# SZU-AdvTech-2024/140-ExtDM-Distribution-Extrapolation-Diffusion-Model-for-Video-Prediction

Hardware: AMD Instinct MI355X
Metric: predicted frames/sec/node (DDPM 1000-step) BAIR 64×64 2→28; FVD parity (higher is better)
Workload: dtype fp32 (f16x3 split-MFMA convs + attention, fp32 accumulate); 1 GPU; BAIR 64x64 ch3 2->28 (tp=14 x 2 rounds), DDPM 1000 steps, Unet3D (multi_w_ref wrapper), LFAE encoder + flow-warp decoder, occlusion map off (eval default); bench_config=bair, global_batch=128, batch_per_gpu=128, sampling_steps=1000, rounds=2, parallelism=clip-shard x1 (+gather to rank 0)

## Files before the change

140-extdm-distribution-extrapolation-diffusion-model-for-video-prediction_amd/csrc/conv_x3.hip:

```cpp
#include <algorithm>
#include <cstdlib>

#include "host_util.h"
#include "kernels.h"

#ifndef EXTDM_X3_LIN
#define EXTDM_X3_LIN 2
#endif
#ifndef EXTDM_X3_BUFX
#define EXTDM_X3_BUFX 1
#endif
#ifndef EXTDM_X3_EXP
#define EXTDM_X3_EXP 0
#endif

namespace extdm {

__device__ int g_x3_range;

namespace {

typedef float f32x16 __attribute__((ext_vector_type(16)));
typedef _Float16 h8 __attribute__((ext_vector_type(8)));
typedef __attribute__((address_space(3))) void* lds_ptr_t;

struct X3Args {
  const float* in0; const float* in1;
  long i0b, i0c, i0t, i1b, i1c, i1t;
  int C0, Cin, H, W, T, P;
  const _Float16* w; const float* wscale; int ncgb;
  float* out; long ob, oc, ot; int Cout;
  int TH, NP, nrow_tiles, RS, XPOS;
  int out_bytes, res_bytes;
  int stats_split;
  const _Float16* xop; long xop_cg, xop_hl;
  float* part; int nsplit;
  float* edge;
  int mfast;
  int mtc;
  int in0_bytes, in1_bytes;
  ConvEpi e;
};

__device__ __forceinline__ float act_apply(float v, int act) {
  switch (act) {
    case ACT_RELU: return v > 0.f ? v : 0.f;
    case ACT_GELU: return 0.5f * v * (1.f + erff(v * 0.70710678118654752f));
    case ACT_SILU: return v / (1.f + expf(-v));
    case ACT_SIGMOID: return 1.f / (1.f + expf(-v));
    default: return v;
  }
}

__device__ __forceinline__ void glds16_asm(const void* gsrc, _Float16* lds) {
  const unsigned dst =
      __builtin_amdgcn_readfirstlane((unsigned)(uintptr_t)(__attribute__((address_space(3))) void*)lds);
  unsigned keep;
  asm volatile("s_mov_b32 %0, m0\n\ts_mov_b32 m0, %2\n\ts_nop 0\n\tglobal_load_lds_dwordx4 %1, off\n\ts_mov_b32 m0, %0"
               : "=&s"(keep)
               : "v"(gsrc), "s"(dst)
               : "memory");
}

__device__ __forceinline__ void bld4_asm(__amdgpu_buffer_rsrc_t rs, int voff, float* lds) {
  const unsigned dst =
      __builtin_amdgcn_readfirstlane((unsigned)(uintptr_t)(__attribute__((address_space(3))) void*)lds);
  unsigned keep;
  asm volatile("s_mov_b32 %0, m0\n\ts_mov_b32 m0, %3\n\ts_nop 0\n\tbuffer_load_dword %1, %2, 0 offen lds\n\ts_mov_b32 m0, %0"
               : "=&s"(keep)
               : "v"(voff), "s"(rs), "s"(dst)
               : "memory");
}

template <int KS, int BN> struct XMaxX3;
template <> struct XMaxX3<7, 256> { static constexpr int v = 560; };
template <> struct XMaxX3<3, 256> { static constexpr int v = 576; };
template <> struct XMaxX3<3, 128> { static constexpr int v = 288; };
template <> struct XMaxX3<1, 128> { static constexpr int v = 128; };
template <> struct XMaxX3<1, 256> { static constexpr int v = 256; };
template <> struct XMaxX3<7, 512> { static constexpr int v = 836; };
template <> struct XMaxX3<3, 512> { static constexpr int v = 800; };
template <> struct XMaxX3<5, 512> { static constexpr int v = 800; };
template <> struct XMaxX3<5, 256> { static constexpr int v = 400; };

template <int KS, int KY, int BM, int BN, int NG, int WN, int NW, int XBUF, bool SPAN, int NS, bool XOP = false,
          bool RGN = false, int SPL = 0, bool PH = false, bool WS = false, bool BX = false, int TT = 0>
__global__ __launch_bounds__(NW * 64) __attribute__((amdgpu_waves_per_eu(NW == 4 && KS == 5 ? 2 : 1))) void conv_x3_kernel(X3Args a) {
  constexpr int NT = NW * 64;
  constexpr int PAD = KS / 2;
  constexpr int CIB = 16 * NG;
  constexpr int MT32 = BM / 32;
  constexpr int KT = TT ? 2 : KS;
  constexpr int STEPS = NG * KT;
  constexpr int AH = STEPS * MT32 * 2 * 512;
  constexpr int AHS = KY * AH;
  constexpr int STG = KT / KY;
  static_assert(KT % KY == 0, "KY must divide the taps");
  static_assert(!TT || (KS == 3 && NG == 1 && BX && SPAN && !XOP && !WS && !PH && SPL == 0), "TT: staged 3x3 geometry");
  constexpr int NSLOT = NS;
  constexpr int WM = NW / WN;
  constexpr int TM = BM / (32 * WM);
  constexpr int TN = BN / (32 * WN);
  static_assert(TM >= 1 && TN >= 1 && WM * WN == NW, "bad tile");
  static_assert(!XOP || (NG == 1 && XBUF == 2 && SPAN), "operand input: one group, two X buffers");

  extern __shared__ __attribute__((aligned(16))) _Float16 smx[];
  static_assert(!WS || (NG == 1 && SPAN && SPL != 2 && NW % 2 == 0), "WS: one group, spanning barriers");
  constexpr bool WSR = WS && !XOP;
  constexpr bool LIN = WSR || ((EXTDM_X3_LIN == 1 || (EXTDM_X3_LIN == 2 && KS >= 5)) && NG == 1 && !XOP);
  const int XPL = ((a.XPOS + (LIN ? 1 : 0) + 63) & ~63) * 8;
  const int XLO = (XOP || LIN) ? 2 * XPL : NG * a.XPOS * 16;
  const int XH = 2 * XLO;
  constexpr int XB = WSR ? 1 : XBUF;
  const int RP = (a.XPOS + 63) & ~63;
  _Float16* As0 = smx;
  _Float16* As1 = smx + AHS;
  _Float16* Xs0 = smx + 2 * AHS;
  _Float16* Xs1 = XB == 2 ? Xs0 + XH : Xs0;
  float* const Xr = reinterpret_cast<float*>(Xs0 + XB * XH);

  const int tid = threadIdx.x, lane = tid & 63, wave = tid >> 6;
  const int wm = wave / WN, wn = wave % WN;
  const int h = lane >> 5, lc = lane & 31;
  int tile, mtile;
  if ((KS == 1 || TT == 1) && a.mfast) {
    const int lin = (int)(blockIdx.x + gridDim.x * blockIdx.y), MT = (int)gridDim.y;
    const int k = lin >> 3;
    mtile = k % MT;
    tile = (lin & 7) + 8 * (k / MT);
  } else {
    tile = (KS == 1 || (gridDim.x & 7)) ? (int)blockIdx.x
                                        : (int)((blockIdx.x & 7) * (gridDim.x >> 3) + (blockIdx.x >> 3));
    mtile = blockIdx.y;
  }
  const int plane0 = (tile / a.nrow_tiles) * a.NP;
  const int row0 = (tile % a.nrow_tiles) * a.TH;

  const int THK = a.TH + KS - 1;
  const int tb = (plane0 * (a.H + KS - 1) + row0) * a.RS;
  const int c0 = SPL == 1 ? (int)blockIdx.z * a.ncgb / a.nsplit : 0;
  const int c1 = SPL == 1 ? ((int)blockIdx.z + 1) * a.ncgb / a.nsplit : a.ncgb;
  const int NIT = c1 * STG;
  const _Float16* wt = a.w + (long)mtile * a.ncgb * KT * AH;
  const int tph = TT == 1 ? mtile / a.mtc : 0;
  const int mbase = (TT == 1 ? mtile - tph * a.mtc : mtile) * BM;
  auto in_phase = [&](int cgb) __attribute__((always_inline)) {
    const int ncb = a.ncgb >> 2;
    return (cgb >= ncb) + (cgb >= 2 * ncb) + (cgb >= 3 * ncb);
  };

  int sg[NSLOT], spos[NSLOT], soff0[NSLOT], soff1[NSLOT];
#pragma unroll
  for (int j = 0; j < NSLOT; ++j) {
    const int sl = tid + NT * j;
    sg[j] = -1; spos[j] = 0; soff0[j] = -1; soff1[j] = -1;
    if (sl < a.XPOS * NG) {
      const int g = sl / a.XPOS, pos = sl - g * a.XPOS;
      const int p = pos / (THK * a.RS);
      const int r2 = pos - p * THK * a.RS;
      const int rr = r2 / a.RS, cc = r2 - rr * a.RS;
      const int q = plane0 + p;
      const int iy = row0 + rr - PAD, ix = cc - PAD;
      sg[j] = g; spos[j] = pos;
      if (q < a.P && iy >= 0 && iy < a.H && ix >= 0 && ix < a.W) {
        const int b = q / a.T, t = q - b * a.T;
        const int ip = TT == 2 ? 4 * iy * a.W + 2 * ix : iy * a.W + ix;
        soff0[j] = (int)((long)b * a.i0b + (long)t * a.i0t) + ip;
        soff1[j] = (int)((long)b * a.i1b + (long)t * a.i1t) + ip;
      }
    }
  }
  float xr[NSLOT][16];
  int range_bad = 0;

  const float* const gin0 = a.in0;
  const float* const gin1 = a.in1;
  const long gi0c = a.i0c, gi1c = a.i1c;
  const int gC0 = a.C0, gCin = a.Cin;
  const bool whole = gC0 % 16 == 0 && gCin % CIB == 0;
  const bool bufx = BX || (EXTDM_X3_BUFX && whole && a.in0_bytes > 0);
  const auto rsx0 = __builtin_amdgcn_make_buffer_rsrc(const_cast<float*>(a.in0), 0, a.in0_bytes, 0x00020000);
  const auto rsx1 = __builtin_amdgcn_make_buffer_rsrc(const_cast<float*>(a.in1), 0, a.in1_bytes, 0x00020000);
  auto load_x_exact = [&](int cgb) __attribute__((always_inline)) {
#if EXTDM_X3_EXP & 2
#pragma unroll
    for (int j = 0; j < NSLOT; ++j)
#pragma unroll
      for (int c = 0; c < 16; ++c) xr[j][c] = 0.f;
    return;
#endif
    if (bufx) {
      const int qin = TT == 2 ? in_phase(cgb) : 0;
      const int cbk = TT == 2 ? cgb - qin * (a.ncgb >> 2) : cgb;
      const int poff = TT == 2 ? ((qin >> 1) * 2 * a.W + (qin & 1)) * 4 : 0;
#pragma unroll
      for (int j = 0; j < NSLOT; ++j) {
        const int ci0 = __builtin_amdgcn_readfirstlane(cbk * CIB + (sg[j] < 0 ? 0 : sg[j]) * 16);
        const bool s1 = ci0 >= gC0;
        const int vo = soff0[j] >= 0 ? (s1 ? soff1[j] : soff0[j]) * 4 : 0x40000000;
        const int cb = s1 ? ci0 - gC0 : ci0;
        const int cs4 = (int)(s1 ? gi1c : gi0c) * 4;
#pragma unroll
        for (int c = 0; c < 16; ++c)
          xr[j][c] = __uint_as_float(__builtin_amdgcn_raw_buffer_load_b32(s1 ? rsx1 : rsx0, vo, (cb + c) * cs4 + poff, 0));
      }
      return;
    }
#pragma unroll
    for (int j = 0; j < NSLOT; ++j) {
      const bool pos_ok = soff0[j] >= 0;
      const int o0 = pos_ok ? soff0[j] : 0, o1 = pos_ok ? soff1[j] : 0;
      const int ci0 = cgb * CIB + (sg[j] < 0 ? 0 : sg[j]) * 16;
      if (whole) {
        const bool s1 = ci0 >= gC0;
        const float* bp = s1 ? gin1 + (long)(ci0 - gC0) * gi1c + o1 : gin0 + (long)ci0 * gi0c + o0;
        const long cs = s1 ? gi1c : gi0c;
#pragma unroll
        for (int c = 0; c < 16; ++c) xr[j][c] = bp[c * cs];
        continue;
      }
#pragma unroll
      for (int c = 0; c < 16; ++c) {
        const int ci = ci0 + c;
        const bool s1 = ci >= gC0;
        int cc = s1 ? ci - gC0 : ci;
        const int cmax = s1 ? gCin - gC0 - 1 : gC0 - 1;
        cc = cc > cmax ? cmax : cc;
        const long off = s1 ? (long)cc * gi1c + o1 : (long)cc * gi0c + o0;
        xr[j][c] = (s1 ? gin1 : gin0)[off];
      }
    }
  };
  auto xmask = [&](int j, int cgb, int c) __attribute__((always_inline)) {
    const int ci = cgb * CIB + (sg[j] < 0 ? 0 : sg[j]) * 16 + c;
    return (soff0[j] >= 0 && ci < gCin) ? 1.f : 0.f;
  };
  auto load_x = [&](int cgb) __attribute__((always_inline)) {
    if (SPAN) {
      load_x_exact(cgb);
      return;
    }
#pragma unroll
    for (int j = 0; j < NSLOT; ++j) {
      const int ci0 = cgb * CIB + sg[j] * 16;
      const bool src1 = ci0 >= a.C0;
      const float* base = src1 ? a.in1 + (long)(ci0 - a.C0) * a.i1c : a.in0 + (long)ci0 * a.i0c;
      const int cs = src1 ? (int)a.i1c : (int)a.i0c;
      const int off = src1 ? soff1[j] : soff0[j];
      const int cend = src1 ? a.Cin : a.C0;
      if (off >= 0 && ci0 + 16 <= cend) {
#pragma unroll
        for (int c = 0; c < 16; ++c) xr[j][c] = base[off + c * cs];
      } else {
#pragma unroll
        for (int c = 0; c < 16; ++c) {
          const int ci = ci0 + c;
          float v = 0.f;
          if (soff0[j] >= 0 && ci < a.Cin)
            v = ci < a.C0 ? a.in0[(long)ci * a.i0c + soff0[j]] : a.in1[(long)(ci - a.C0) * a.i1c + soff1[j]];
          xr[j][c] = v;
        }
      }
    }
  };
  _Float16* const xdummy = Xs0 + XB * XH + (WSR ? 2 * 16 * RP : 0);
  auto store_x = [&](_Float16* Xs, int cgb) __attribute__((always_inline)) {
#pragma unroll
    for (int j = 0; j < NSLOT; ++j) {
      if (!SPAN && sg[j] < 0) continue;
      float v[16];
#pragma unroll
      for (int c = 0; c < 16; ++c) {
        float r = xr[j][c];
        if (SPAN) {
          asm volatile("" : "+v"(r));
          if (!bufx) r *= xmask(j, cgb, c);
        }
        v[c] = r;
      }
      unsigned hw[8], lw[8];
      float am = 0.f;
#pragma unroll
      for (int c = 0; c < 8; ++c) {
        split2s(v[2 * c], v[2 * c + 1], hw[c], lw[c]);
        amax2(am, v[2 * c], v[2 * c + 1]);
      }
      range_bad |= am >= 65504.f;
      const h8 hi0 = __builtin_bit_cast(h8, u32x4{hw[0], hw[1], hw[2], hw[3]});
      const h8 hi1 = __builtin_bit_cast(h8, u32x4{hw[4], hw[5], hw[6], hw[7]});
      const h8 lo0 = __builtin_bit_cast(h8, u32x4{lw[0], lw[1], lw[2], lw[3]});
      const h8 lo1 = __builtin_bit_cast(h8, u32x4{lw[4], lw[5], lw[6], lw[7]});
      const bool used = sg[j] >= 0;
      if (LIN) {
        _Float16* d = Xs + (used ? spos[j] : XPL / 8 - 1) * 8;
        *reinterpret_cast<h8*>(d) = hi0;
        *reinterpret_cast<h8*>(d + XPL) = hi1;
        *reinterpret_cast<h8*>(d + 2 * XPL) = lo0;
        *reinterpret_cast<h8*>(d + 3 * XPL) = lo1;
        continue;
      }
      const int sw = (spos[j] >> 3) & 1;
      _Float16* dh = used ? Xs + ((long)sg[j] * a.XPOS + spos[j]) * 16 : xdummy;
      _Float16* dl = used ? dh + XLO : xdummy + 16;
      *reinterpret_cast<h8*>(dh + 8 * sw) = hi0;
      *reinterpret_cast<h8*>(dh + 8 * (sw ^ 1)) = hi1;
      *reinterpret_cast<h8*>(dl + 8 * sw) = lo0;
      *reinterpret_cast<h8*>(dl + 8 * (sw ^ 1)) = lo1;
    }
  };
  constexpr int NPIECE = AHS / 512;
  const int wave_u = __builtin_amdgcn_readfirstlane(wave);
  auto load_a = [&](int it, _Float16* As) {
#if EXTDM_X3_EXP & 8
    return;
#endif
    const _Float16* src = wt + (long)it * AHS;
    if (WS && wave_u >= NW / 2) return;
    for (int pc = wave_u; pc < NPIECE; pc += (WS ? NW / 2 : NW)) {
      if (SPAN) glds16_asm(src + pc * 512 + lane * 8, As + pc * 512);
      else
        __builtin_amdgcn_global_load_lds((const void*)(src + pc * 512 + lane * 8), (lds_ptr_t)(As + pc * 512), 16, 0,
                                         0);
    }
  };

  auto dma_x = [&](int cgb, _Float16* Xs) __attribute__((always_inline)) {
    const _Float16* src = a.xop + (long)cgb * a.xop_cg + (long)tb * 8;
    const int npc = (a.XPOS + 63) >> 6;
    if (WS && wave_u < NW / 2) return;
    for (int pc = WS ? wave_u - NW / 2 : wave_u; pc < 4 * npc; pc += (WS ? NW / 2 : NW)) {
      const int pl = pc / npc, k = pc - pl * npc;
      glds16_asm(src + (pl >> 1) * a.xop_hl + (pl & 1) * (a.xop_hl >> 1) + k * 512 + lane * 8,
                 Xs + pl * XPL + k * 512);
    }
  };

  constexpr int NXW = NW / 2;
  constexpr int WCH = WSR ? (XMaxX3<KS, BN>::v + 64 * NXW - 1) / (64 * NXW) : 1;
  int xo0[WCH], xo1[WCH];
  if (WSR) {
    const int xw = wave - NXW;
#pragma unroll
    for (int i = 0; i < WCH; ++i) {
      const int pos = (xw + NXW * i) * 64 + lane;
      xo0[i] = 0x40000000; xo1[i] = 0x40000000;
      if (xw >= 0 && pos < a.XPOS) {
        const int p = pos / (THK * a.RS), r2 = pos - p * THK * a.RS;
        const int rr = r2 / a.RS, cc = r2 - rr * a.RS;
        const int q = plane0 + p, iy = row0 + rr - PAD, ix = cc - PAD;
        if (q < a.P && iy >= 0 && iy < a.H && ix >= 0 && ix < a.W) {
          const int b = q / a.T, t = q - b * a.T;
          xo0[i] = (int)(((long)b * a.i0b + (long)t * a.i0t) + iy * a.W + ix) * 4;
          xo1[i] = (int)(((long)b * a.i1b + (long)t * a.i1t) + iy * a.W + ix) * 4;
        }
      }
    }
  }
  auto dma_raw = [&](int cgb) __attribute__((always_inline)) {
    if (!WSR || wave_u < NXW) return;
    const int xw = wave_u - NXW;
#pragma unroll 4
    for (int c = 0; c < 16; ++c) {
      const int ci = cgb * 16 + c;
      const bool s1 = ci >= gC0;
      const int co = (int)((s1 ? ci - gC0 : ci) * (s1 ? gi1c : gi0c)) * 4;
#pragma unroll
      for (int i = 0; i < WCH; ++i) {
        const int k = xw + NXW * i;
        if (k * 64 < a.XPOS) bld4_asm(s1 ? rsx1 : rsx0, (s1 ? xo1[i] : xo0[i]) + co, Xr + c * RP + k * 64);
      }
    }
  };
  auto split_raw = [&]() __attribute__((always_inline)) {
    for (int p = tid; p < a.XPOS; p += NT) {
      float v[16];
#pragma unroll
      for (int c = 0; c < 16; ++c) v[c] = Xr[c * RP + p];
      unsigned hw[8], lw[8];
      float am = 0.f;
#pragma unroll
      for (int c = 0; c < 8; ++c) {
        split2s(v[2 * c], v[2 * c + 1], hw[c], lw[c]);
        amax2(am, v[2 * c], v[2 * c + 1]);
      }
      range_bad |= am >= 65504.f;
      _Float16* d = Xs0 + p * 8;
      *reinterpret_cast<h8*>(d) = __builtin_bit_cast(h8, u32x4{hw[0], hw[1], hw[2], hw[3]});
      *reinterpret_cast<h8*>(d + XPL) = __builtin_bit_cast(h8, u32x4{hw[4], hw[5], hw[6], hw[7]});
      *reinterpret_cast<h8*>(d + 2 * XPL) = __builtin_bit_cast(h8, u32x4{lw[0], lw[1], lw[2], lw[3]});
      *reinterpret_cast<h8*>(d + 3 * XPL) = __builtin_bit_cast(h8, u32x4{lw[4], lw[5], lw[6], lw[7]});
    }
  };

  int bpos[TN];
#pragma unroll
  for (int j = 0; j < TN; ++j) {
    const int n = (wn * TN + j) * 32 + lc;
    const int p = n / (a.TH * a.W);
    const int r = (n / a.W) % a.TH;
    const int c = n % a.W;
    bpos[j] = (p * THK + r) * a.RS + c;
    if (TT == 1) bpos[j] += (tph >> 1) * a.RS + (tph & 1);
  }

  f32x16 acc[TM][TN];
#pragma unroll
  for (int i = 0; i < TM; ++i)
#pragma unroll
    for (int j = 0; j < TN; ++j)
#pragma unroll
      for (int r = 0; r < 16; ++r) acc[i][j][r] = 0.f;

  float* const ep_sc = reinterpret_cast<float*>(xdummy + 32);
  float* const ep_bi = ep_sc + BM;
  if (tid < BM) {
    const int m = mbase + tid;
    const int mc = m < a.Cout ? m : a.Cout - 1;
    ep_sc[tid] = a.wscale[mc];
    ep_bi[tid] = a.e.bias ? a.e.bias[mc] : 0.f;
  }
  if (SPL == 2) {
    const long per = (long)TM * TN * 16 * NT;
    const float* pp = a.part + ((long)mtile * gridDim.x + tile) * per + tid;
    const long zs = (long)gridDim.y * gridDim.x * per;
    for (int z = 0; z < a.nsplit; ++z)
#pragma unroll
      for (int i = 0; i < TM; ++i)
#pragma unroll
        for (int j = 0; j < TN; ++j)
#pragma unroll
          for (int r = 0; r < 16; ++r) acc[i][j][r] += pp[z * zs + (long)((i * TN + j) * 16 + r) * NT];
    __syncthreads();
  } else if (XOP) {
    dma_x(c0, Xs0);
    load_a(c0 * STG, As0);
  } else if (WSR) {
    dma_raw(c0);
    load_a(c0 * STG, As0);
  } else {
    load_x(c0);
    load_a(c0 * STG, As0);
    store_x(Xs0, c0);
  }
  if (SPL == 2) {
  } else if (SPAN) asm volatile("s_waitcnt vmcnt(0) lgkmcnt(0)\n\ts_barrier" ::: "memory");
  else __syncthreads();
  if (WSR && SPL != 2) {
    split_raw();
    asm volatile("s_waitcnt lgkmcnt(0)\n\ts_barrier" ::: "memory");
  }
  auto export_edges = [&](const _Float16* Xs, int cgb) __attribute__((always_inline)) {
    const int nrec = a.NP * 4 * a.W;
    for (int r = tid; r < nrec; r += NT) {
      const int pp = r / (4 * a.W), rem = r - pp * 4 * a.W, line = rem / a.W, jj = rem - line * a.W;
      const int q = plane0 + pp;
      const int iy = line == 0 ? 0 : (line == 1 ? a.H - 1 : jj);
      const int ix = line == 2 ? 0 : (line == 3 ? a.W - 1 : jj);
      if (q >= a.P || iy < row0 || iy >= row0 + a.TH) continue;
      const int pos = (pp * THK + iy - row0 + PAD) * a.RS + ix + PAD;
      h8 h0, h1, l0, l1;
      if (LIN) {
        const _Float16* xh = Xs + (long)pos * 8;
        h0 = *reinterpret_cast<const h8*>(xh);
        h1 = *reinterpret_cast<const h8*>(xh + XPL);
        l0 = *reinterpret_cast<const h8*>(xh + 2 * XPL);
        l1 = *reinterpret_cast<const h8*>(xh + 3 * XPL);
      } else {
        const int sw = (pos >> 3) & 1;
        const _Float16* xh = Xs + (long)pos * 16;
        h0 = *reinterpret_cast<const h8*>(xh + 8 * sw);
        h1 = *reinterpret_cast<const h8*>(xh + 8 * (sw ^ 1));
        l0 = *reinterpret_cast<const h8*>(xh + XLO + 8 * sw);
        l1 = *reinterpret_cast<const h8*>(xh + XLO + 8 * (sw ^ 1));
      }
      float v[16];
#pragma unroll
      for (int c = 0; c < 8; ++c) {
        v[c] = (float)h0[c] + (float)l0[c] * (1.f / X3_LO_UP);
        v[8 + c] = (float)h1[c] + (float)l1[c] * (1.f / X3_LO_UP);
      }
      float4* d = reinterpret_cast<float4*>(a.edge + (((long)q * 4 + line) * a.W + jj) * a.Cin + cgb * CIB);
#pragma unroll
      for (int c = 0; c < 4; ++c) d[c] = make_float4(v[4 * c], v[4 * c + 1], v[4 * c + 2], v[4 * c + 3]);
    }
  };
  auto stage = [&](int cgb, int kb, bool more) __attribute__((always_inline)) {
    const int it = cgb * STG + kb;
    const int itr = it - c0 * STG, cr = cgb - c0;
    const _Float16* Ast = (itr & 1) ? As1 : As0;
    const _Float16* Xs = (cr & 1) ? Xs1 : Xs0;
    if (PH && !XOP && kb == 0 && a.edge && mtile == 0) export_edges(Xs, cgb);
    if (it + 1 < NIT) load_a(it + 1, (itr & 1) ? As0 : As1);
    const bool pre = (kb == 0) && more;
    int torg = 0;
    if (TT == 2) {
      const int qin = in_phase(cgb);
      torg = (1 - (qin >> 1)) * a.RS + 1 - (qin & 1);
    }
    if (SPAN) __builtin_amdgcn_sched_barrier(0);
    if (pre) {
      if (XOP) dma_x(cgb + 1, (cr & 1) ? Xs0 : Xs1);
      else if (WSR) dma_raw(cgb + 1);
// ... 55 lines not shown
        if (SPAN) asm volatile("s_waitcnt lgkmcnt(0)\n\ts_barrier" ::: "memory");
        else __syncthreads();
      }
      store_x((cr & 1) ? Xs0 : Xs1, cgb + 1);
    }
    if (SPAN) {
      if (!XOP && pre && STG > 1) {
        asm volatile("s_waitcnt vmcnt(%0) lgkmcnt(0)\n\ts_barrier" ::"n"(16 * NSLOT) : "memory");
      } else {
        asm volatile("s_waitcnt vmcnt(0) lgkmcnt(0)\n\ts_barrier" ::: "memory");
      }
    } else {
      __syncthreads();
    }
  };
  auto channel_block = [&](int cgb, bool more) __attribute__((always_inline)) {
    stage(cgb, 0, more);
    if (STG > 3) {
#pragma unroll 1
      for (int kb = 1; kb < STG; ++kb) stage(cgb, kb, more);
    } else {
#pragma unroll
      for (int kb = 1; kb < STG; ++kb) stage(cgb, kb, more);
    }
  };
  if (SPL != 2) {
    for (int cgb = c0; cgb + 1 < c1; ++cgb) channel_block(cgb, true);
    channel_block(c1 - 1, false);
  }
  if (range_bad) atomicOr(&g_x3_range, 1);
  if (SPL == 1) {
    const long per = (long)TM * TN * 16 * NT;
    float* pp = a.part + (((long)blockIdx.z * gridDim.y + mtile) * gridDim.x + tile) * per + tid;
#pragma unroll
    for (int i = 0; i < TM; ++i)
#pragma unroll
      for (int j = 0; j < TN; ++j)
#pragma unroll
        for (int r = 0; r < 16; ++r) pp[(long)((i * TN + j) * 16 + r) * NT] = acc[i][j][r];
    return;
  }

  const bool has_res = a.e.res != nullptr;
  const bool res_gn = RGN && has_res;
  const bool has_post = a.e.post_scale != nullptr, post_pc = a.e.post_per_channel != 0;
  const int act = a.e.act;
  const bool do_stats = a.e.stats != nullptr;
  float* const red = reinterpret_cast<float*>(smx);
  const auto rs_out = __builtin_amdgcn_make_buffer_rsrc(a.out, 0, a.out_bytes, 0x00020000);
  const auto rs_res = __builtin_amdgcn_make_buffer_rsrc(const_cast<float*>(a.e.res), 0, a.res_bytes, 0x00020000);
#pragma unroll
  for (int i = 0; i < TM; ++i) {
    int mrow[16];
    float scl[16], bia[16];
    float st_s[4] = {0.f, 0.f, 0.f, 0.f}, st_q[4] = {0.f, 0.f, 0.f, 0.f};
#pragma unroll
    for (int k = 0; k < 4; ++k) {
      const int ml = (wm * TM + i) * 32 + 8 * k + 4 * h;
      const float4 s4 = *reinterpret_cast<const float4*>(ep_sc + ml);
      const float4 b4 = *reinterpret_cast<const float4*>(ep_bi + ml);
      scl[4 * k] = s4.x; scl[4 * k + 1] = s4.y; scl[4 * k + 2] = s4.z; scl[4 * k + 3] = s4.w;
      bia[4 * k] = b4.x; bia[4 * k + 1] = b4.y; bia[4 * k + 2] = b4.z; bia[4 * k + 3] = b4.w;
    }
#pragma unroll
    for (int r16 = 0; r16 < 16; ++r16) {
      const int m = mbase + (wm * TM + i) * 32 + (r16 & 3) + 8 * (r16 >> 2) + 4 * h;
      mrow[r16] = m < a.Cout ? m : a.Cout - 1;
    }
#pragma unroll
    for (int j = 0; j < TN; ++j) {
      const int n = (wn * TN + j) * 32 + lc;
      const int p = n / (a.TH * a.W);
      const int r = (n / a.W) % a.TH;
      const int c = n % a.W;
      const int q0 = plane0 + p, row0q = row0 + r;
      const bool valid = q0 < a.P && row0q < a.H;
      const int q = valid ? q0 : 0, row = valid ? row0q : 0;
      const int b = q / a.T, t = q - b * a.T;
      const int ph = TT == 1 ? tph : (mtile * BM + (wm * TM + i) * 32) / 64;
      const int pix = (PH || TT == 1) ? (2 * row + (ph >> 1)) * (2 * a.W) + 2 * c + (ph & 1) : row * a.W + c;
      float v[16];
#pragma unroll
      for (int r16 = 0; r16 < 16; ++r16) v[r16] = acc[i][j][r16] * scl[r16] + bia[r16];
      if (has_res) {
        const int rbase = (int)((long)b * a.e.res_sb + (long)t * a.e.res_st) + pix;
        float rv[16];
#pragma unroll
        for (int r16 = 0; r16 < 16; ++r16)
          rv[r16] = __uint_as_float(__builtin_amdgcn_raw_buffer_load_b32(
              rs_res, (rbase + (PH ? mrow[r16] - ph * 64 : mrow[r16]) * (int)a.e.res_sc) * 4, 0, 0));
        if (res_gn) {
#pragma unroll
          for (int r16 = 0; r16 < 16; ++r16) {
            const float2 ab = a.e.res_aff[b * a.Cout + mrow[r16]];
            const float w = rv[r16] * ab.x + ab.y;
            rv[r16] = w / (1.f + expf(-w));
          }
        }
#pragma unroll
        for (int r16 = 0; r16 < 16; ++r16) v[r16] += rv[r16];
      }
      if (has_post) {
        float ps[16], pt[16];
#pragma unroll
        for (int r16 = 0; r16 < 16; ++r16) {
          const int pi = post_pc ? mrow[r16] : b * a.Cout + mrow[r16];
          ps[r16] = a.e.post_scale[pi];
          pt[r16] = a.e.post_shift[pi];
        }
#pragma unroll
        for (int r16 = 0; r16 < 16; ++r16) v[r16] = v[r16] * ps[r16] + pt[r16];
      }
      if (act != ACT_NONE) {
#pragma unroll
        for (int r16 = 0; r16 < 16; ++r16) v[r16] = act_apply(v[r16], act);
      }
      const int obase = (int)((long)b * a.ob + (long)t * a.ot) + pix;
#pragma unroll
      for (int r16 = 0; r16 < 16; ++r16) {
        const int m = mbase + (wm * TM + i) * 32 + (r16 & 3) + 8 * (r16 >> 2) + 4 * h;
        const bool ok = valid && m < a.Cout;
        const int off = ok ? (obase + (PH ? m - ph * 64 : m) * (int)a.oc) * 4 : a.out_bytes;
#if EXTDM_X3_EXP & 4
        if (v[r16] == 12345.678f)
#endif
        __builtin_amdgcn_raw_buffer_store_b32(__float_as_uint(v[r16]), rs_out, off, 0, 0);
        if (do_stats) {
          const float x = ok ? v[r16] : 0.f;
          st_s[r16 >> 2] += x;
          st_q[r16 >> 2] += x * x;
        }
      }
    }
    if (do_stats) {
#pragma unroll
      for (int k = 0; k < 4; ++k) {
        float s_ = st_s[k], q_ = st_q[k];
#pragma unroll
        for (int off = 32; off >= 1; off >>= 1) {
          s_ += __shfl_xor(s_, off);
          q_ += __shfl_xor(q_, off);
        }
        if (lane == 0) {
          red[(wave * TM * 4 + i * 4 + k) * 2] = s_;
          red[(wave * TM * 4 + i * 4 + k) * 2 + 1] = q_;
        }
      }
    }
  }
  if (do_stats) {
    __syncthreads();
    const int G = a.e.stats_groups, Cg = a.Cout / G;
    const int ngrp = BM / Cg;
    if (tid < ngrp) {
      const int g = mtile * ngrp + tid;
      if (g < G) {
        double s_ = 0.0, q_ = 0.0;
        for (int kb = tid * (Cg / 8); kb < (tid + 1) * (Cg / 8); ++kb) {
          const int wmk = kb / (TM * 4), ik = kb % (TM * 4);
          for (int wn_ = 0; wn_ < WN; ++wn_) {
            const int w_ = wmk * WN + wn_;
            s_ += (double)red[(w_ * TM * 4 + ik) * 2];
            q_ += (double)red[(w_ * TM * 4 + ik) * 2 + 1];
          }
        }
        const int bq = plane0 / a.T;
        const int slot = ((plane0 % a.T) / a.NP) * a.nrow_tiles + tile % a.nrow_tiles;
        double* pp = a.e.stats + (((long)bq * G + g) * a.stats_split + slot) * 2;
        pp[0] = s_;
        pp[1] = q_;
      }
    }
  }
}

bool x3_bufx_ok(const X3Args& a, int cib) {
  static const bool off = env_flag("EXTDM_X3_NO_BX");
  return !off && EXTDM_X3_BUFX && a.C0 % 16 == 0 && a.Cin % cib == 0 && a.in0_bytes > 0;
}

template <int KS, int KY, int BM, int BN, int NG, int WN, int NW, int XBUF, bool SPAN, int NS, bool XOP = false,
          bool RGN = false, int SPL = 0, bool PH = false, bool WS = false>
void launch_sp(hipStream_t s, const X3Args& a, unsigned ntiles) {
  constexpr int AH = KY * NG * KS * (BM / 32) * 2 * 512;
  constexpr bool WSR = WS && !XOP;
// ... 18 lines not shown
  if (SPL != 2) {
    auto tf = [](bool v) { return v ? "true" : "false"; };
    note_kernel("conv_x3_kernel<%d, %d, %d, %d, %d, %d, %d, %d, %s, %d, %s, %s, %d, %s, %s, %s>", KS, KY, BM, BN, NG, WN,
                NW, XBUF, tf(SPAN), NS, tf(XOP), tf(RGN), SPL, tf(PH), tf(WS), tf(bx));
  }
  if (bx)
    hipLaunchKernelGGL((conv_x3_kernel<KS, KY, BM, BN, NG, WN, NW, XBUF, SPAN, NS, XOP, RGN, SPL, PH, WS, BXV>), grid, dim3(NW * 64), lds, s, a);
  else
    hipLaunchKernelGGL((conv_x3_kernel<KS, KY, BM, BN, NG, WN, NW, XBUF, SPAN, NS, XOP, RGN, SPL, PH, WS>), grid, dim3(NW * 64), lds, s, a);
}

template <int KS, int KY, int BM, int BN, int NG, int WN, int NW, int XBUF, bool SPAN>
void launch_ns(hipStream_t s, const X3Args& a, unsigned ntiles) {
  constexpr int XMAX = XMaxX3<KS, BN>::v;
  constexpr int NT = NW * 64;
  static_assert((XMAX * NG + NT - 1) / NT <= 3, "more than three staging slots");
  const int need = (a.XPOS * NG + NT - 1) / NT;
  if constexpr (XMAX * NG <= NT) launch_sp<KS, KY, BM, BN, NG, WN, NW, XBUF, SPAN, 1>(s, a, ntiles);
  else if constexpr (XMAX * NG <= 2 * NT) {
    if (need <= 1) launch_sp<KS, KY, BM, BN, NG, WN, NW, XBUF, SPAN, 1>(s, a, ntiles);
    else launch_sp<KS, KY, BM, BN, NG, WN, NW, XBUF, SPAN, 2>(s, a, ntiles);
  } else {
    if (need <= 1) launch_sp<KS, KY, BM, BN, NG, WN, NW, XBUF, SPAN, 1>(s, a, ntiles);
    else if (need == 2) launch_sp<KS, KY, BM, BN, NG, WN, NW, XBUF, SPAN, 2>(s, a, ntiles);
    else launch_sp<KS, KY, BM, BN, NG, WN, NW, XBUF, SPAN, 3>(s, a, ntiles);
  }
}

constexpr int kLongKBlocks = 128;
int split_slices_longk(const X3Args& a) {
  static const bool on = [] { const char* v = getenv("EXTDM_X3_LONGK"); return !(v && v[0] == '0'); }();
  if (!on || a.ncgb < kLongKBlocks || a.P < 1) return 0;
  const long nwg16 = (16L * a.T + a.NP - 1) / a.NP * a.nrow_tiles * ((a.Cout + 255) / 256);
  const double blk_us = 1.74;
  const double part_us = (double)a.Cout * (16.0 * a.T * a.H * a.W) * 8.0 / 1.5e6;
  int best = 1;
  double bc = 1e300;
  for (int S = 1; S <= a.ncgb / 16; ++S) {
    const double c = (double)((nwg16 * S + 255) / 256) * ((a.ncgb + S - 1) / S) * blk_us + (S > 1 ? S * part_us : 0.0);
    if (c < bc * 0.999) { bc = c; best = S; }
  }
  return best >= 2 ? best : 0;
}

int split_slices(const X3Args& a, unsigned ntiles, long max_wg, long max_total, int bm = 128) {
  static const bool off = env_flag("EXTDM_NO_SPLITK");
  (void)ntiles;
  if (off || a.ncgb < 4 || a.P < 1) return 0;
  if (bm == 256 && a.ncgb >= kLongKBlocks) return split_slices_longk(a);
  const long nwg64 = (64L * a.T + a.NP - 1) / a.NP * a.nrow_tiles * ((a.Cout + bm - 1) / bm);
  if (nwg64 >= max_wg) return 0;
  const int S = (int)std::min<long>(a.ncgb / 2, max_total / nwg64);
  return S >= 2 ? S : 0;
}
size_t split_bytes(const X3Args& a, unsigned ntiles, int S) {
  return S ? (size_t)S * ntiles * ((a.Cout + 127) / 128) * 128 * 128 * sizeof(float) : 0;
}
bool x3_split256() {
  static const bool on = [] { const char* v = getenv("EXTDM_X3_SPLIT256"); return !(v && v[0] == '0'); }();
  return on;
}
bool split_k(X3Args& a, unsigned ntiles, const ConvEpi& e, long max_wg, long max_total, int bm = 128) {
  const int S = split_slices(a, ntiles, max_wg, max_total, bm);
  if (!S || !e.split_ws || split_bytes(a, ntiles, S) > e.split_ws_bytes) return false;
  a.part = e.split_ws;
  a.nsplit = S;
  return true;
}

enum { kWsPhase = 1, kWsStaged64 = 2, kWsOp64 = 4, kWsOp128 = 8 };
bool x3_ws(int fam) {
  static const int mask = [] { const char* v = getenv("EXTDM_X3_WS"); return v ? atoi(v) : 0; }();
  return (mask & fam) != 0;
}
bool x3_ws_raw_ok(const X3Args& a, int fam) {
  return x3_ws(fam) && a.C0 % 16 == 0 && a.Cin % 16 == 0 && a.in0_bytes > 0;
}

int x3_v3() {
  static const int v3 = [] { const char* v = getenv("EXTDM_X3_V3"); return v ? atoi(v) : 0; }();
  return v3;
}

bool x3_w128_4(const X3Args& a, bool xop) {
  static const int w = [] { const char* v = getenv("EXTDM_X3_W128"); return v ? atoi(v) : 4; }();
  if (w == 8) return false;
  constexpr size_t AH = 3 * 4 * 2 * 512;
  const size_t xlo = xop ? (size_t)((a.XPOS + 63) & ~63) * 16
                         : (EXTDM_X3_LIN == 1 ? (size_t)((a.XPOS + 1 + 63) & ~63) * 16 : (size_t)a.XPOS * 16);
  return (2 * AH + 2 * 2 * xlo + 32 + 4 * 128) * sizeof(_Float16) <= 80 * 1024;
}
void x3_split128(bool four, long& max_wg, long& max_total) {
  static const long* t4 = [] {
    static long v[2] = {256, 512};
    if (const char* e = getenv("EXTDM_X3_SPLIT4")) sscanf(e, "%ld,%ld", &v[0], &v[1]);
    return v;
  }();
  if (four) { max_wg = t4[0]; max_total = t4[1]; } else { max_wg = 128; max_total = 256; }
}

template <int KS, int KY, int BM, int BN, int NG, int WN, int NW, int XBUF>
void launch(hipStream_t s, const X3Args& a, unsigned ntiles) {
  static const bool nospan = env_flag("EXTDM_X3_NOSPAN");
  if (nospan) launch_ns<KS, KY, BM, BN, NG, WN, NW, XBUF, false>(s, a, ntiles);
  else launch_ns<KS, KY, BM, BN, NG, WN, NW, XBUF, true>(s, a, ntiles);
}

}

X3Tile x3_tile(int ks, int cout) {
  X3Tile t{};
  if (ks == 7) {
    static const int bn7 = [] { const char* v = getenv("EXTDM_X3_BN7"); return v ? atoi(v) : 512; }();
    t.bm = 64; t.bn = bn7 == 256 ? 256 : 512; t.ng = 1;
  }
  else if (ks == 5) {
    static const int bm5 = [] { const char* v = getenv("EXTDM_FEA_BM"); return v ? atoi(v) : 128; }();
    if (bm5 == 128) { t.bm = 128; t.bn = 256; } else { t.bm = 64; t.bn = 512; }
    t.ng = 1;
  }
  else if (ks == 3) {
    static const int bn3 = [] { const char* v = getenv("EXTDM_X3_BN3"); return v ? atoi(v) : 256; }();
    if (cout <= 64) { t.bm = 64; t.bn = bn3 == 512 ? 512 : 256; } else { t.bm = 128; t.bn = 128; }
    t.ng = 1;
  }
  else if (ks == 1) {
    static const int bm1 = [] { const char* v = getenv("EXTDM_X3_BM1"); return v ? atoi(v) : 256; }();
    t.bm = cout <= 64 ? 64 : ((bm1 == 256 && cout % 256 == 0) ? 256 : 128);
    t.bn = 128; t.ng = 2;
  }
  return t;
}

namespace {

bool x3_setup(const View& out, const View& in0, const View* in1, const PackedW& w, const ConvEpi& epi, X3Args& a,
              unsigned& ntiles, int* stats_slots) {
  if (stats_slots) *stats_slots = 0;
  if (!w.wx || w.mode != MODE_CONV) return false;
  const int ks = w.KH;
  const int H = in0.H, W = in0.W;
  const X3Tile tl{w.xbm, w.xbn, w.xng};
  if (out.H != H || out.W != W || W > tl.bn || tl.bn % W != 0) return false;
  if ((long)in0.B * in0.sb > (1L << 31) || (in1 && (long)in1->B * in1->sb > (1L << 31))) return false;
  a = X3Args{};
  a.TH = std::min(H, tl.bn / W);
  if (tl.bn % (a.TH * W) != 0) return false;
  a.NP = tl.bn / (a.TH * W);
  a.RS = W + ks - 1;
  a.XPOS = a.NP * (a.TH + ks - 1) * a.RS;
  const int xmax = tl.bn == 512 ? (ks == 7 ? 836 : 800)
                                 : (ks == 7 ? 560 : (ks == 5 ? 400 : (ks == 3 ? (tl.bn == 256 ? 576 : 288) : (tl.bn == 256 ? 256 : 128))));
  if (a.XPOS > xmax) return false;
  a.in0 = in0.p; a.i0b = in0.sb; a.i0c = in0.sc; a.i0t = in0.st; a.C0 = in0.C;
  if (in1) { a.in1 = in1->p; a.i1b = in1->sb; a.i1c = in1->sc; a.i1t = in1->st; a.Cin = in0.C + in1->C; }
  else { a.in1 = in0.p; a.i1b = in0.sb; a.i1c = in0.sc; a.i1t = in0.st; a.Cin = in0.C; }
  a.H = H; a.W = W; a.T = out.T; a.P = out.B * out.T;
  a.w = reinterpret_cast<const _Float16*>(w.wx); a.wscale = w.xscale; a.ncgb = w.xncgb;
  a.out = out.p; a.ob = out.sb; a.oc = out.sc; a.ot = out.st; a.Cout = out.C;
  a.nrow_tiles = (H + a.TH - 1) / a.TH;
  a.e = epi;
  auto extent = [&](long sb, long sc, long st, int C) {
    return ((long)(out.B - 1) * sb + (long)(C - 1) * sc + (long)(out.T - 1) * st + (long)H * W) * 4;
  };
  const long ob = extent(out.sb, out.sc, out.st, out.C);
  const long rb = epi.res ? extent(epi.res_sb, epi.res_sc, epi.res_st, out.C) : 0;
  if (ob >= (1L << 31) - 4 || rb >= (1L << 31) - 4) return false;
  a.out_bytes = (int)ob;
  a.res_bytes = (int)rb;
  ntiles = (unsigned)(((a.P + a.NP - 1) / a.NP) * a.nrow_tiles);
  {
    auto ext_in = [&](const View& v) {
      return ((long)(v.B - 1) * v.sb + (long)(v.C - 1) * v.sc + (long)(v.T - 1) * v.st + (long)v.H * v.W) * 4;
    };
    const long e0 = ext_in(in0), e1 = in1 ? ext_in(*in1) : e0;
    const bool ok = e0 < (1L << 30) && e1 < (1L << 30) && (tl.ng == 1 || a.XPOS % 64 == 0);
    a.in0_bytes = ok ? (int)e0 : 0;
    a.in1_bytes = ok ? (int)e1 : 0;
  }
  if (epi.stats) {
    const int G = epi.stats_groups, Cg = G > 0 ? out.C / G : 0;
    const int split = (out.T / std::max(a.NP, 1)) * a.nrow_tiles;
    const bool ok = G > 0 && out.C % G == 0 && Cg % 8 == 0 && tl.bm % Cg == 0 && out.T % a.NP == 0 &&
                    split >= 1 && split <= 64;
    if (ok) {
      a.stats_split = split;
      if (stats_slots) *stats_slots = split;
    } else {
      a.e.stats = nullptr;
    }
  }
  return true;
}

}

bool x3_mfast(const X3Args& a, const X3Tile& tl, unsigned ntiles) {
  static const bool off = env_flag("EXTDM_X3_NO_MFAST");
  static const long cap = [] { const char* v = getenv("EXTDM_X3_MFAST_KB"); return (v ? atol(v) : 3584L) * 1024; }();
  const long mt = (a.Cout + tl.bm - 1) / tl.bm;
  return !off && mt > 1 && ntiles % 8 == 0 && mt * tl.bm * (long)a.Cin * 4 <= cap;
}

bool x3_bn256(const View& out, const PackedW& w, const ConvEpi& epi) {
  static const int bn1 = [] { const char* v = getenv("EXTDM_X3_BN1"); return v ? atoi(v) : 256; }();
  if ((bn1 != 256 && bn1 != 64) || w.KH != 1 || w.xbm != 256 || w.xbn != 128 || epi.res_aff) return false;
  static const bool longk = [] { const char* v = getenv("EXTDM_X3_LONGK"); return !(v && v[0] == '0'); }();
  if (longk && w.xncgb >= kLongKBlocks) return false;
  const int H = out.H, W = out.W;
  if (W > 256 || 256 % W != 0) return false;
  const int TH = std::min(H, 256 / W);
  if (256 % (TH * W) != 0) return false;
  const long NP = 256 / (TH * W), nrow = (H + TH - 1) / TH;
  const long Bref = bn1 == 64 ? 64L : (long)out.B;
  const long nwg = (Bref * out.T + NP - 1) / NP * nrow * ((out.C + 255) / 256);
  return nwg >= 192;
}

bool conv_x3_forward(hipStream_t s, const View& out, const View& in0, const View* in1, const PackedW& w0,
                     const ConvEpi& epi, int* stats_slots) {
  PackedW wt = w0;
  if (x3_bn256(out, w0, epi)) wt.xbn = 256;
  const PackedW& w = wt;
  X3Args a;
  unsigned ntiles = 0;
  if (!x3_setup(out, in0, in1, w, epi, a, ntiles, stats_slots)) return false;
  const int ks = w.KH;
  const X3Tile tl{w.xbm, w.xbn, w.xng};
  if (ks == 1) a.mfast = x3_mfast(a, tl, ntiles);
  if (epi.res_aff) {
    if (ks != 1 || !epi.res || tl.bn != 128) return false;
    if (tl.bm == 64) launch_sp<1, 1, 64, 128, 2, 4, 4, 2, true, 1, false, true>(s, a, ntiles);
    else if (tl.bm == 128) launch_sp<1, 1, 128, 128, 2, 2, 4, 2, true, 1, false, true>(s, a, ntiles);
    else if (tl.bm == 256) launch_sp<1, 1, 256, 128, 2, 2, 8, 2, true, 1, false, true>(s, a, ntiles);
    else return false;
    return true;
  }
  if (tl.bn == 512) {
    static const int nw7 = [] { const char* v = getenv("EXTDM_X3_NW7"); return v ? atoi(v) : 8; }();
    if (ks == 7 && tl.bm == 64 && nw7 != 16) launch<7, 1, 64, 512, 1, 8, 8, 1>(s, a, ntiles);
    else if (ks == 7 && tl.bm == 64) launch<7, 1, 64, 512, 1, 8, 16, 1>(s, a, ntiles);
    else if (ks == 3 && tl.bm == 64) launch<3, 1, 64, 512, 1, 8, 16, 1>(s, a, ntiles);
    else return false;
    return true;
  }
  if (ks == 7 && tl.bm == 64) launch<7, 1, 64, 256, 1, 4, 8, 2>(s, a, ntiles);
  else if (ks == 3 && tl.bm == 64) {
    if (x3_v3() == 1) launch<3, 3, 64, 256, 1, 4, 8, 2>(s, a, ntiles);
    else if (x3_ws_raw_ok(a, kWsStaged64)) launch_sp<3, 1, 64, 256, 1, 4, 4, 2, true, 1, false, false, 0, false, true>(s, a, ntiles);
    else launch<3, 1, 64, 256, 1, 4, 4, 2>(s, a, ntiles);
  }
  else if (ks == 3 && tl.bm == 128) {
    const bool four = x3_w128_4(a, false);
    long mw, mt;
    x3_split128(four, mw, mt);
    if (four && split_k(a, ntiles, epi, mw, mt)) {
      launch_sp<3, 1, 128, 128, 1, 2, 4, 2, true, 1, false, false, 1>(s, a, ntiles);
      launch_sp<3, 1, 128, 128, 1, 2, 4, 2, true, 1, false, false, 2>(s, a, ntiles);
    } else if (!four && split_k(a, ntiles, epi, mw, mt)) {
      launch_sp<3, 1, 128, 128, 1, 2, 8, 2, true, 1, false, false, 1>(s, a, ntiles);
      launch_sp<3, 1, 128, 128, 1, 2, 8, 2, true, 1, false, false, 2>(s, a, ntiles);
    } else if (four) {
      launch<3, 1, 128, 128, 1, 2, 4, 2>(s, a, ntiles);
    } else {
      launch<3, 1, 128, 128, 1, 2, 8, 2>(s, a, ntiles);
    }
  }
  else if (ks == 1 && tl.bm == 64) launch<1, 1, 64, 128, 2, 4, 4, 2>(s, a, ntiles);
  else if (ks == 1 && tl.bm == 256 && tl.bn == 256) launch<1, 1, 256, 256, 2, 2, 8, 2>(s, a, ntiles);
  else if (ks == 1 && tl.bm == 256) {
    if (x3_split256() && split_k(a, ntiles, epi, 256, 256, 256)) {
      launch_sp<1, 1, 256, 128, 2, 2, 8, 2, true, 1, false, false, 1>(s, a, ntiles);
      launch_sp<1, 1, 256, 128, 2, 2, 8, 2, true, 1, false, false, 2>(s, a, ntiles);
    } else {
      launch<1, 1, 256, 128, 2, 2, 8, 2>(s, a, ntiles);
    }
  }
  else if (ks == 1 && tl.bm == 128) {
    if (split_k(a, ntiles, epi, 384, 512)) {
      launch_sp<1, 1, 128, 128, 2, 2, 4, 2, true, 1, false, false, 1>(s, a, ntiles);
      launch_sp<1, 1, 128, 128, 2, 2, 4, 2, true, 1, false, false, 2>(s, a, ntiles);
    } else {
      launch<1, 1, 128, 128, 2, 2, 4, 2>(s, a, ntiles);
    }
  }
  else return false;
  return true;
}

bool conv_x3_phase_forward(hipStream_t s, const View& out, const View& in, const PackedW& w, const ConvEpi& epi,
                           float* edge, bool dry) {
  if (!w.wx || w.mode != MODE_CONV || w.KH != 5 || !((w.xbm == 64 && w.xbn == 512) || (w.xbm == 128 && w.xbn == 256)) ||
      w.M != 4 * out.C || out.C != 64)
    return false;
  if (out.H != 2 * in.H || out.W != 2 * in.W || out.B != in.B || out.T != in.T || in.C * 25 != w.K) return false;
  View og = out;
  og.H = in.H; og.W = in.W; og.C = w.M;
  X3Args a;
  unsigned ntiles = 0;
  ConvEpi e = epi;
  e.stats = nullptr;
  static const int bn = [] { const char* v = getenv("EXTDM_FEA_TILE"); return v ? atoi(v) : 512; }();
  PackedW wt = w;
// ... 233 lines not shown
```

140-extdm-distribution-extrapolation-diffusion-model-for-video-prediction_amd/csrc/kernels.h:

```cpp
#pragma once
#include <hip/hip_runtime.h>
#include <stdint.h>

namespace extdm {

__device__ __forceinline__ float split_src(float v) {
  asm("" : "+v"(v));
  return v;
}

typedef unsigned u32x4 __attribute__((ext_vector_type(4)));

__device__ __forceinline__ void split2(float a, float b, unsigned& hi, unsigned& lo) {
  float da, db;
  asm("v_cvt_pk_f16_f32 %0, %4, %5\n\t"
      "v_fma_mix_f32 %2, -%0, 1.0, %4 op_sel_hi:[1,0,0]\n\t"
      "v_fma_mix_f32 %3, -%0, 1.0, %5 op_sel:[1,0,0] op_sel_hi:[1,0,0]\n\t"
      "v_cvt_pk_f16_f32 %1, %2, %3"
      : "=&v"(hi), "=v"(lo), "=&v"(da), "=&v"(db)
      : "v"(a), "v"(b));
}
typedef float f32x2s_t __attribute__((ext_vector_type(2)));
__device__ __forceinline__ void split2s(float a, float b, unsigned& hi, unsigned& lo) {
  const f32x2s_t V = (f32x2s_t){a, b} * 2048.f;
// ... 15 lines not shown
__device__ __forceinline__ f2 pair(float a, float b) { f2 v = {a, b}; return v; }
__device__ __forceinline__ f2 splat(float a) { f2 v = {a, a}; return v; }
__device__ __forceinline__ void split2c(float a, float b, f16x2_t& hi, f16x2_t& lo) {
  hi = __builtin_convertvector((f32x2_t){a, b}, f16x2_t);
  const float one = split_src(1.0f);
  const float la = __builtin_fmaf(-(float)hi.x, one, a);
  const float lb = __builtin_fmaf(-(float)hi.y, one, b);
  lo = __builtin_convertvector((f32x2_t){la, lb}, f16x2_t);
}
__device__ __forceinline__ void split2m(float a, float b, f16x2_t& hi, f16x2_t& lo) {
  hi = __builtin_convertvector((f32x2_t){a, b}, f16x2_t);
  const float one = split_src(1.0f);
  lo.x = (_Float16)__builtin_fmaf(-(float)hi.x, one, a);
  lo.y = (_Float16)__builtin_fmaf(-(float)hi.y, one, b);
}
__device__ __forceinline__ void amax2(float& m, float a, float b) {
  asm("v_max3_f32 %0, |%1|, |%2|, %0" : "+v"(m) : "v"(a), "v"(b));
}

void note_kernel(const char* fmt, ...);
const char* noted_kernel();

struct View {
  float* p = nullptr;
  int B = 0, C = 0, T = 0, H = 0, W = 0;
  long sb = 0, sc = 0, st = 0;
  int HW() const { return H * W; }
  long numel() const { return (long)B * C * T * H * W; }
  View frames(int t0, int n) const {
    View v = *this; v.p = p + (long)t0 * st; v.T = n; return v;
  }
  View chans(int c0, int n) const {
    View v = *this; v.p = p + (long)c0 * sc; v.C = n; return v;
  }
};

inline View cf_view(float* p, int B, int C, int T, int H, int W) {
  View v; v.p = p; v.B = B; v.C = C; v.T = T; v.H = H; v.W = W;
  v.st = (long)H * W; v.sc = (long)T * H * W; v.sb = (long)C * T * H * W; return v;
}
inline View tm_view(float* p, int B, int C, int T, int H, int W) {
  View v; v.p = p; v.B = B; v.C = C; v.T = T; v.H = H; v.W = W;
  v.sc = (long)H * W; v.st = (long)C * H * W; v.sb = (long)C * T * H * W; return v;
}

enum Act { ACT_NONE = 0, ACT_RELU = 1, ACT_GELU = 2, ACT_SILU = 3, ACT_SIGMOID = 4 };
enum ConvMode { MODE_CONV = 0, MODE_DECONV = 1, MODE_UP2 = 2 };

struct PackedW {
  float* w = nullptr;
  int K = 0, M = 0, Kpad = 0, Mpad = 0, KH = 1, KW = 1, mode = MODE_CONV;
  float* wh = nullptr;
  int hstages = 0, hbm = 0;
  void* wx = nullptr;
  float* xscale = nullptr;
  int xbm = 0, xbn = 0, xng = 0, xncgb = 0;
  void* tx = nullptr;
  float* tscale = nullptr;
  int tbm = 0, tbn = 0, tncb = 0;
  void* gx = nullptr;
  float* gscale = nullptr;
  int gbm = 0, gnkt = 0;
  void* gxt = nullptr;
  int gnkt_t = 0;
  float* wv = nullptr;
  int vcot = 0;
};

inline int conv_bm(int M) { return M <= 32 ? 32 : ((M <= 64 || M % 128 != 0) ? 64 : 128); }

struct ConvEpi {
  const float* bias = nullptr;
  const float* res = nullptr;
  long res_sb = 0, res_sc = 0, res_st = 0;
  const float* post_scale = nullptr;
  const float* post_shift = nullptr;
  int post_per_channel = 0;
  int act = ACT_NONE;
  double* stats = nullptr;
  int stats_groups = 0;
  const float2* res_aff = nullptr;
  float* split_ws = nullptr;
  size_t split_ws_bytes = 0;
};

int halo_ch(int ks, int bm);
bool conv_halo_forward(hipStream_t s, const View& out, const View& in0, const View* in1, const PackedW& w,
                       const ConvEpi& epi);

struct X3Tile { int bm, bn, ng; };
X3Tile x3_tile(int ks, int cout);

bool conv_x3_forward(hipStream_t s, const View& out, const View& in0, const View* in1, const PackedW& w,
                     const ConvEpi& epi, int* stats_slots = nullptr);
bool conv_x3_covers(const View& out, const View& in0, const View* in1, const PackedW& w);
size_t conv_x3_split_bytes(const View& out, const View& in0, const View* in1, const PackedW& w);
size_t conv_x3_op_split_bytes(const View& out, const PackedW& w, int C);
struct X3Op {
  _Float16* p = nullptr;
  int B = 0, C = 0, T = 0, H = 0, W = 0, pad = 0;
};
size_t x3op_halves(int B, int C, int T, int H, int W, int pad);
bool conv_x3_op_supported(const View& out, const PackedW& w, int C, int pad);
bool conv_x3_forward_op(hipStream_t s, const View& out, const X3Op& in, const PackedW& w, const ConvEpi& epi,
                        int* stats_slots = nullptr);
bool conv_x3_phase_forward(hipStream_t s, const View& out, const View& in, const PackedW& w, const ConvEpi& epi,
                           float* edge = nullptr, bool dry = false);
struct FeaSideArgs {
  const float* e;
  int C, L, T, P;
  const _Float16* w; const float* wscale;
  float* out; long ob, oc, ot; int OH, OW, Co;
  int out_bytes, pair;
  int* range;
};
struct FeaCornerArgs {
  const float* e;
  int C, L, T, P;
  const float* dw;
  float* out; long ob, oc, ot; int OH, OW, Co;
};
inline size_t fea_edge_floats(int P, int C, int L) { return (size_t)P * 4 * L * C; }
bool fea_edges_supported(int C, int Co, int L);
bool fea_edges_forward(hipStream_t s, const View& out, const float* edge, int C, const void* side_w,
                       const float* side_scale, const float* corner_w, bool dry = false);
bool conv_x3_updown_forward(hipStream_t s, const View& out, const View& in0, const View* in1, const PackedW& w,
                            int stride, int pad, const ConvEpi& epi);
void x3_range_reset(hipStream_t s);
bool pw_x3_forward(hipStream_t s, const View& out, const View& in, const PackedW& w, const ConvEpi& e);
size_t frame_metrics_workspace(int nframes, int C, int H);
void frame_metrics(hipStream_t s, const float* a, const float* b, int N, int T, int C, int H, int W, long sN, long sT,
                   long sC, double* psnr, double* ssim, double* work);
int* x3_range_ptr();
int x3_range_read(hipStream_t s);

int conv_forward(hipStream_t s, const View& out, const View& in0, const View* in1, const PackedW& w,
                 int stride, int pad, const ConvEpi& epi);

void groupnorm_silu(hipStream_t s, const View& x, const View& out, int groups, const float* gamma,
                    const float* beta, const float* film, int film_row, int film_nt, const int* t_batch,
                    const View* res, double* partials, int given_split = 0);
void groupnorm_silu_x3op(hipStream_t s, const View& x, const X3Op& out, int groups, const float* gamma,
                         const float* beta, const float* film, int film_row, int film_nt, const int* t_batch,
                         double* partials, int given_split = 0);
const float2* groupnorm_affine(hipStream_t s, const View& x, int groups, const float* gamma, const float* beta,
                               double* partials, int given_split = 0);

void channel_ln(hipStream_t s, const View& out, const View& in0, const View* in1, const float* gamma);
void temporal_prologue(hipStream_t s, const View& x, const float* gamma, const float* lw, const float* lb,
                       const View& z, const View& r);

struct AttnGeom {
  int mode;
  int D, H, W;
  int ws0, ws1, ws2;
  int ss0, ss1, ss2;
  int Dp, Hp, Wp;
  int per;
};
__host__ __device__ inline int temporal_slots(const AttnGeom& g) { return g.per ? g.per : (g.D <= 16 ? 16 : 32); }
bool attention_core(hipStream_t s, const View& qkv, const View& o, const AttnGeom& g, int heads, int dim_head,
                    const float* bias_dense, int bstride, const float* rope_cos, const float* rope_sin, float q_scale,
                    bool bf16);
void window_attention(hipStream_t s, const View& qkv, const View& o, const AttnGeom& g, int heads,
                      const float* bias_dense , const float* rope_cos,
                      const float* rope_sin , float q_scale);
bool temporal_attention64(hipStream_t s, const View& qkv, const View& o, const AttnGeom& g, int heads, int dim_head,
                          const float* bias64, const float* rope_cos, const float* rope_sin, float q_scale);
bool fused_attn_supported(int C, int ntok, int dim_head, int heads);
bool stw_fused(hipStream_t s, const View& x, const AttnGeom& g, int heads, int dim_head, const float* gamma,
               const float* wqkv, const float* wp, const float* bp, const float* bias_dense, int bstride,
               const float* rcos, const float* rsin, float q_scale);
bool temporal_fused(hipStream_t s, const View& x, const View& out, const AttnGeom& g, int heads, int dim_head,
                    const float* gamma, const float* ln_w, const float* ln_b, const float* wqkv, const float* wout,
                    const float* bias_dense, int bstride, const float* rcos, const float* rsin, float q_scale);
bool attn_x3_supported(int C, int ntok, int dim_head, int heads);
int attn_x3_unit_halves(int C);
bool stw_x3(hipStream_t s, const View& x, const AttnGeom& g, int heads, int dim_head, const float* gamma,
            const void* wpk, const float* wsc, const float* bp, const float* mbias, int npat,
            const float* rcos, const float* rsin, float q_scale, bool bf16);
bool stw64_x3_supported(int C, int ntok, int dim_head, int heads);
bool stw64_x3(hipStream_t s, const View& x, const AttnGeom& g, int heads, int dim_head, const float* gamma,
              const void* wpk, const float* wsc, const float* bp, const float* mbias, int npat, const float* rcos,
              const float* rsin, float q_scale, bool bf16);
bool temporal_x3(hipStream_t s, const View& x, const View& out, const AttnGeom& g, int heads, int dim_head,
                 const float* gamma, const float* ln_w, const float* ln_b, const void* wpk, const float* wsc,
                 const float* mbias, const float* rcos, const float* rsin, float q_scale, bool bf16);
bool temporal64_x3_supported(int C, int frames, int dim_head, int heads);
bool temporal64_x3(hipStream_t s, const View& x, const View& out, const AttnGeom& g, int heads, int dim_head,
                   const float* gamma, const float* ln_w, const float* ln_b, const void* wpk, const float* wsc,
                   const float* mbias, const float* rcos, const float* rsin, float q_scale, bool bf16);
struct XPathArgs {
  const float* x; long xb, xc, xt;
  int T, L, F, LP;
  float* out; long ob, oc, ot; int Cout;
  const _Float16* w; const float* rscale; const float* cbias;
  const float* add; long ab, ac, at;
  int FG, ngroups, gtiles, xcd;
  int tile_start[50];
  int tile_last[50];
};
bool xpath_x3_forward(hipStream_t s, const View& out, const View& x, const void* w, const float* rscale,
                      const float* cbias, const View* add = nullptr);
int xpad_size(int L);
void xpad_forward(hipStream_t s, const View& xpad, const View& x);
struct NoisePoolArgs {
  const float* x; long xb, xc, xt;
  int T, L, F, LP;
  float* out; long ob, oc, ot; int Cout;
  const _Float16* w; const float* rscale; const float* bias;
  const float* add; long ab, ac, at;
};
bool noise_pool_x3_forward(hipStream_t s, const View& out, const View& x, const void* w, const float* rscale,
                           const float* bias);
bool conv7c3_x3_forward(hipStream_t s, const View& out, const View& x, const void* w, const float* rscale,
                        const float* bias, const View* add);
int narrow_cot(int KS, int M);
bool conv_narrow_forward(hipStream_t s, const View& out, const View& in0, const View* in1, const PackedW& w,
                         int stride, int pad, const ConvEpi& epi);
bool conv_gemm_x3_forward(hipStream_t s, const View& out, const View& in0, const View* in1, const PackedW& w,
                          int stride, int pad, const ConvEpi& epi);
void cross_attention(hipStream_t s, const float* q, const float* k, const float* v, float* o, int B, int C,
                     int heads, int NQ, int NK);
bool cross_attention_x3(hipStream_t s, const float* q, const float* k, const float* v, float* o, int B, int C,
                        int heads, int NQ, int NK);
size_t cross_kv_halves(int B, int C, int heads, int NK);
bool cross_kv_split(hipStream_t s, const float* k, const float* v, _Float16* kvp, int B, int C, int heads, int NK);
bool cross_attention_x3p(hipStream_t s, const float* q, const _Float16* kvp, float* o, int B, int C, int heads, int NQ,
                         int NK);

void copy_view(hipStream_t s, const View& dst, const View& src);
void maxpool_hw2(hipStream_t s, const View& dst, const View& src);
void bilinear_frames(hipStream_t s, const View& dst, const View& a, const View& b, int t_split);
void adaptor_stats(hipStream_t s, const View& x, float* mean, float* std_, double* partials);
void adaptor_normalize(hipStream_t s, const View& dst, const View& src, const float* mean, const float* std_);
void zero_pad_frames(hipStream_t s, const View& x);

struct StepCoef {
  float sra, srm1;
  float c1, c2, sigma;
  int t;
  int use_noise;
  int kind;
};
void sampler_step(hipStream_t s, float* x, const float* eps, int B, int n, const StepCoef* coefs,
                  const int* step_ctr, const float* noise , uint64_t seed, int sample_base,
                  int round, int k_lo, int k_hi, float q_w, float* thresh_out);
size_t sampler_sel_bytes(int B, int n);
void sampler_step_mw(hipStream_t s, float* x, const float* eps, int B, int n, const StepCoef* coefs, int* step_ctr,
                     const float* noise, uint64_t seed, int sample_base, int round, int k_lo, int k_hi, float q_w,
                     float* thresh_out, unsigned* ws, int* t_next, int nsteps);
void sampler_step_t(hipStream_t s, float* x, const float* eps, int B, int n, const StepCoef* coefs, const float* noise,
                    int k_lo, int k_hi, float q_w, float* thresh_out, unsigned* ws);
void q_sample(hipStream_t s, float* xt, const float* x0, const float* noise, float* noise_out, int B, int n,
              const float2* qc, uint64_t seed, int sample_base, int round);
int loss_chunks(int n);
void x0_loss(hipStream_t s, const float* xt, const float* eps, const float* noise, int B, int n, const StepCoef* coefs,
             int loss_type, bool clip, int k_lo, int k_hi, float q_w, float* pred_x0, double* part, double* loss_sum,
             float* thresh_out, unsigned* ws);
void abs_diff_sum(hipStream_t s, const float* a, const float* b, int B, int n, double* part, double* sums);
void fill_normal(hipStream_t s, float* x, int B, int n, uint64_t seed, int sample_base, int round, int stream_id);
void set_t_from_step(hipStream_t s, int* t_batch, int B, const StepCoef* coefs, const int* step_ctr);
void incr_counter(hipStream_t s, int* ctr);
void t_to_int(hipStream_t s, const int64_t* t, int* t_batch, int B);

void warp_blend(hipStream_t s, float* out, const float* src, int N, int C, int S, const float* flow,
                const float* occ, int T, int fh, int fw, const float* prev);
void affine_relu(hipStream_t s, float* out, const float* in, const float* a, const float* b, int N, int C, int HW);
void avgpool2(hipStream_t s, float* out, const float* in, int planes, int Ho, int Wo);

void warp_frames(hipStream_t s, float* out, const float* src, const float* flow, int B, int C, int T, int S,
                 int fh, int fw, long out_sb, long out_sc, long out_st);

void aa_down(hipStream_t s, float* out, const float* in, const float* w, int N, int C, int H, int W, int k,
             int step);
void region_stats(hipStream_t s, const float* logits, int NR, int h, int w, float temperature, float* heat,
                  float* shift, float* covar, float* affine, float* u, float* sv);
void bg_head(hipStream_t s, const float* feat, int N, int Cin, int HW, const float* fw, const float* fb, int nout,
             int bg_type, float* out);
void sparse_motion(hipStream_t s, const float* src, const float* dshift, const float* dcov, const float* daff,
                   const float* sshift, const float* scov, const float* saff, const float* bg, float* motion,
                   float* pin, int N, int R, int C, int h, int w, int use_cov, int use_def, int revert, float var);
void flow_combine(hipStream_t s, const float* logits, const float* motion, int N, int K, int h, int w, float* flow);

}
```

140-extdm-distribution-extrapolation-diffusion-model-for-video-prediction_amd/csrc/norm.hip:

```cpp
#include "kernels.h"
#include <stdexcept>

namespace extdm {

namespace {

__device__ __forceinline__ double wave_sum(double v) {
#pragma unroll
  for (int o = 32; o > 0; o >>= 1) v += __shfl_xor(v, o);
  return v;
}

__device__ __forceinline__ void block_sum2(double& a, double& b, double* sh) {
  a = wave_sum(a);
  b = wave_sum(b);
  const int w = threadIdx.x >> 6, l = threadIdx.x & 63;
  __syncthreads();
  if (l == 0) { sh[w] = a; sh[4 + w] = b; }
  __syncthreads();
  a = sh[0] + sh[1] + sh[2] + sh[3];
  b = sh[4] + sh[5] + sh[6] + sh[7];
}

struct V5 {
// ... 291 lines not shown
      bad |= fabsf(w) >= 65504.f;
      const _Float16 a = (_Float16)w;
      hi[e >> 3][e & 7] = a;
      lo[e >> 3][e & 7] = (_Float16)((w - (float)a) * X3_LO_UP);
    }
    if (tpos < n) {
      _Float16* d = ob + (long)tpos * 8;
      *reinterpret_cast<h8*>(d) = hi[0];
      *reinterpret_cast<h8*>(d + c8s) = hi[1];
      *reinterpret_cast<h8*>(d + hl_stride) = lo[0];
      *reinterpret_cast<h8*>(d + hl_stride + c8s) = lo[1];
    }
  }
  if (bad) atomicOr(range_flag, 1);
}

__device__ __forceinline__ float ld2(const float* p0, long b0, long c0s, int C0, const float* p1, long b1,
                                     long c1s, int c) {
  return c < C0 ? p0[b0 + (long)c * c0s] : p1[b1 + (long)(c - C0) * c1s];
}

__global__ __launch_bounds__(256) void channel_ln4_kernel(float* out, long osb, long osc, long ost,
                                                          const float* p0, long sb0, long sc0, long st0, int C0,
                                                          const float* p1, long sb1, long sc1, long st1, int C,
                                                          int T, int HW, int B, const float* gamma) {
  __shared__ double red[8][32][4], red2[8][32][4];
  __shared__ float stat[2][32][4];
  const int q = threadIdx.x & 31, grp = threadIdx.x >> 5;
  const long nq = (long)B * T * HW / 4;
  const long idx = (long)blockIdx.x * 32 + q;
  const bool ok = idx < nq;
  const long pix = (ok ? idx : 0) * 4;
  const int hw = (int)(pix % HW);
  const int t = (int)((pix / HW) % T);
  const int b = (int)(pix / ((long)HW * T));
  const long b0 = (long)b * sb0 + (long)t * st0 + hw;
  const long b1 = (long)b * sb1 + (long)t * st1 + hw;
  auto ld4 = [&](int c) __attribute__((always_inline)) {
    return c < C0 ? *reinterpret_cast<const float4*>(p0 + b0 + (long)c * sc0)
                  : *reinterpret_cast<const float4*>(p1 + b1 + (long)(c - C0) * sc1);
  };
  double s[4] = {0.0, 0.0, 0.0, 0.0}, ss[4] = {0.0, 0.0, 0.0, 0.0};
  if (ok) {
#pragma unroll 4
    for (int c = grp; c < C; c += 8) {
      const float4 v = ld4(c);
      const double d[4] = {v.x, v.y, v.z, v.w};
#pragma unroll
      for (int k = 0; k < 4; ++k) { s[k] += d[k]; ss[k] += d[k] * d[k]; }
    }
  }
#pragma unroll
  for (int k = 0; k < 4; ++k) { red[grp][q][k] = s[k]; red2[grp][q][k] = ss[k]; }
  __syncthreads();
  if (threadIdx.x < 128) {
    const int qq = threadIdx.x >> 2, k = threadIdx.x & 3;
    double tt = 0.0, t2 = 0.0;
    for (int i = 0; i < 8; ++i) { tt += red[i][qq][k]; t2 += red2[i][qq][k]; }
    const double mean = tt / C;
    double var = t2 / C - mean * mean;
    if (var < 0) var = 0;
    stat[0][qq][k] = (float)mean;
    stat[1][qq][k] = sqrtf((float)var + 1e-5f);
  }
  __syncthreads();
  if (!ok) return;
  float m[4], den[4];
#pragma unroll
  for (int k = 0; k < 4; ++k) { m[k] = stat[0][q][k]; den[k] = stat[1][q][k]; }
  const long ob = (long)b * osb + (long)t * ost + hw;
#pragma unroll 4
  for (int c = grp; c < C; c += 8) {
    const float4 v = ld4(c);
    const float g = gamma[c];
    float4 o;
    o.x = (v.x - m[0]) / den[0] * g;
    o.y = (v.y - m[1]) / den[1] * g;
    o.z = (v.z - m[2]) / den[2] * g;
    o.w = (v.w - m[3]) / den[3] * g;
    *reinterpret_cast<float4*>(out + ob + (long)c * osc) = o;
  }
}

__global__ __launch_bounds__(256) void channel_ln_kernel(float* out, long osb, long osc, long ost,
                                                         const float* p0, long sb0, long sc0, long st0, int C0,
                                                         const float* p1, long sb1, long sc1, long st1, int C,
                                                         int T, int HW, int B, const float* gamma) {
  __shared__ double red[8][33], red2[8][33];
  __shared__ float stat[2][32];
  const int px = threadIdx.x & 31, grp = threadIdx.x >> 5;
  const long idx = (long)blockIdx.x * 32 + px;
  const long npix = (long)B * T * HW;
  const bool ok = idx < npix;
  const long id2 = ok ? idx : 0;
  const int hw = (int)(id2 % HW);
  const int t = (int)((id2 / HW) % T);
  const int b = (int)(id2 / ((long)HW * T));
  const long b0 = (long)b * sb0 + (long)t * st0 + hw;
  const long b1 = (long)b * sb1 + (long)t * st1 + hw;
  double s = 0.0, ss = 0.0;
  if (ok)
    for (int c = grp; c < C; c += 8) {
      const double v = ld2(p0, b0, sc0, C0, p1, b1, sc1, c);
      s += v;
      ss += v * v;
    }
  red[grp][px] = s;
  red2[grp][px] = ss;
  __syncthreads();
  if (threadIdx.x < 32) {
    double tt = 0.0, t2 = 0.0;
    for (int i = 0; i < 8; ++i) { tt += red[i][threadIdx.x]; t2 += red2[i][threadIdx.x]; }
    const double mean = tt / C;
    double var = t2 / C - mean * mean;
    if (var < 0) var = 0;
    stat[0][threadIdx.x] = (float)mean;
    stat[1][threadIdx.x] = sqrtf((float)var + 1e-5f);
  }
  __syncthreads();
  if (!ok) return;
  const float m = stat[0][px], den = stat[1][px];
  const long ob = (long)b * osb + (long)t * ost + hw;
  for (int c = grp; c < C; c += 8) {
    const float x = ld2(p0, b0, sc0, C0, p1, b1, sc1, c);
    out[ob + (long)c * osc] = (x - m) / den * gamma[c];
  }
}

__global__ __launch_bounds__(256) void temporal_prologue_kernel(const float* x, long sb, long sc, long st, int C,
                                                                int T, int HW, int B, const float* gamma,
                                                                const float* lw, const float* lb, float* z,
                                                                long zsb, long zsc, long zst, float* r, long rsb,
                                                                long rsc, long rst) {
  const long idx = (long)blockIdx.x * 256 + threadIdx.x;
  const long npix = (long)B * T * HW;
  if (idx >= npix) return;
  const int hw = (int)(idx % HW);
  const int t = (int)((idx / HW) % T);
  const int b = (int)(idx / ((long)HW * T));
  const float* xp = x + (long)b * sb + (long)t * st + hw;
  double s = 0.0;
  for (int c = 0; c < C; ++c) s += xp[(long)c * sc];
  const float m = (float)(s / C);
  double v2 = 0.0;
  for (int c = 0; c < C; ++c) {
    const double d = (double)xp[(long)c * sc] - (double)(s / C);
    v2 += d * d;
  }
  const float den = sqrtf((float)(v2 / C) + 1e-5f);
  double sy = 0.0;
  for (int c = 0; c < C; ++c) sy += (double)((xp[(long)c * sc] - m) / den * gamma[c]);
  const double my = sy / C;
  double vy = 0.0;
  for (int c = 0; c < C; ++c) {
    const double d = (double)((xp[(long)c * sc] - m) / den * gamma[c]) - my;
    vy += d * d;
  }
  const float m2 = (float)my;
  const float rstd2 = 1.0f / sqrtf((float)(vy / C) + 1e-5f);
  float* zp = z + (long)b * zsb + (long)t * zst + hw;
  float* rp = r + (long)b * rsb + (long)t * rst + hw;
  for (int c = 0; c < C; ++c) {
    const float xv = xp[(long)c * sc];
    const float y = (xv - m) / den * gamma[c];
    zp[(long)c * zsc] = (y - m2) * rstd2 * lw[c] + lb[c];
    rp[(long)c * rsc] = xv + y;
// ... 158 lines not shown
                                                           long bsc, long bst, int tsplit, int C, int nbc, int Ho,
                                                           int Wo, int Hi, int Wi, int vec) {
  __shared__ float pl[BPLS * 1024];
  const int t = blockIdx.y;
  const int bc0 = blockIdx.x * BPLS;
  const int np = nbc - bc0 < BPLS ? nbc - bc0 : BPLS;
  const int HWi = Hi * Wi;
  for (int k = threadIdx.x; k < np * HWi; k += 256) {
    const int j = k / HWi, e = k - j * HWi;
    const int bc = bc0 + j;
    const int b = bc / C, c = bc - b * C;
    const float* p = t < tsplit ? a + off5(asb, asc, ast, b, c, t, 0) : bb + off5(bsb, bsc, bst, b, c, t - tsplit, 0);
    pl[j * HWi + e] = p[e];
  }
  __syncthreads();
  const int n4 = Ho * Wo / 4;
  for (int k = threadIdx.x; k < np * n4; k += 256) {
    const int j = k / n4, q = k - j * n4;
    const int bc = bc0 + j;
    const int b = bc / C, c = bc - b * C;
    const int y = 4 * q / Wo, x = 4 * q - y * Wo;
    int y0, y1;
    float ly0, ly1;
    lin_idx(y, Hi, Ho, y0, y1, ly0, ly1);
    const float* r0 = pl + j * HWi + y0 * Wi;
    const float* r1 = pl + j * HWi + y1 * Wi;
    float v[4];
#pragma unroll
    for (int u = 0; u < 4; ++u) {
      int x0, x1;
      float lx0, lx1;
      lin_idx(x + u, Wi, Wo, x0, x1, lx0, lx1);
      v[u] = ly0 * (lx0 * r0[x0] + lx1 * r0[x1]) + ly1 * (lx0 * r1[x0] + lx1 * r1[x1]);
    }
    float* o = d + off5(dsb, dsc, dst_, b, c, t, y * Wo + x);
    if (vec) {
      *reinterpret_cast<float4*>(o) = make_float4(v[0], v[1], v[2], v[3]);
    } else {
#pragma unroll
      for (int u = 0; u < 4; ++u) o[u] = v[u];
    }
  }
}

__global__ __launch_bounds__(256) void adaptor_stats_kernel(const float* x, long sb, long sc, long st, int C, int T,
                                                            int HW, float* mean_out, float* std_out) {
  const int bc = blockIdx.x;
  const int b = bc / C, c = bc % C;
  const float* p = x + (long)b * sb + (long)c * sc;
  const int n = T * HW;
  double s = 0.0, dummy = 0.0;
  const int t0 = threadIdx.x / HW, hw0 = threadIdx.x - t0 * HW;
  const int dt = 256 / HW, dhw = 256 - dt * HW;
  {
    int t = t0, hw = hw0;
    for (int e = threadIdx.x; e < n; e += 256) {
      s += p[(long)t * st + hw];
      t += dt; hw += dhw;
      if (hw >= HW) { hw -= HW; ++t; }
    }
  }
  __shared__ double sh[8];
  block_sum2(s, dummy, sh);
  const double mean = s / n;
  double v2 = 0.0;
  dummy = 0.0;
  {
    int t = t0, hw = hw0;
    for (int e = threadIdx.x; e < n; e += 256) {
      const double d = p[(long)t * st + hw] - mean;
      v2 += d * d;
      t += dt; hw += dhw;
      if (hw >= HW) { hw -= HW; ++t; }
    }
  }
  __syncthreads();
  block_sum2(v2, dummy, sh);
  if (threadIdx.x == 0) {
    mean_out[bc] = (float)mean;
    std_out[bc] = sqrtf((float)(v2 / (n - 1)) + 1e-5f);
  }
}

__global__ __launch_bounds__(256) void adaptor_norm_kernel(float* d, long dsb, long dsc, long dst_, const float* s,
                                                           long ssb, long ssc, long sst, int C, int T, int HW,
                                                           const float* mean, const float* std_) {
  const int e = blockIdx.x * 256 + threadIdx.x;
  if (e >= T * HW) return;
  const int bc = blockIdx.y;
  const int b = bc / C, c = bc - b * C;
  const int t = e / HW, hw = e - t * HW;
  d[off5(dsb, dsc, dst_, b, c, t, hw)] = (s[off5(ssb, ssc, sst, b, c, t, hw)] - mean[bc]) / std_[bc];
}

__global__ __launch_bounds__(256) void zero_pad_frames_kernel(float* p, long sb, long last, long len4) {
  const long e = (long)blockIdx.x * 256 + threadIdx.x;
  if (e >= len4) return;
  const int r = blockIdx.y;
  float4* row = reinterpret_cast<float4*>(p + (long)(r >> 1) * sb + (r & 1) * last);
  row[e] = make_float4(0.f, 0.f, 0.f, 0.f);
}

inline unsigned nblk(long n) { return (unsigned)((n + 255) / 256); }

}

namespace {

bool al16(const void* p) { return ((uintptr_t)p & 15) == 0; }

int gn_statistics(hipStream_t s, const View& x, int groups, double* partials, int given_split) {
  if (x.st != x.HW() || x.sc != (long)x.T * x.HW() || x.C % groups != 0)
    throw std::invalid_argument("groupnorm_silu: input must be [B][C][T][H][W] with contiguous (C, T, H, W) "
                                "per sample and C divisible by the group count");
  if (given_split > 0) return given_split;
  const int Cg = x.C / groups;
  const long L = (long)Cg * x.T * x.HW();
  int split = (int)((L + 32767) / 32768);
  if (split < 1) split = 1;
  if (split > 64) split = 64;
  if (L % 4 == 0 && al16(x.p) && x.sb % 4 == 0 && x.sc % 4 == 0) {
    long chunk = (L + 63) / 64;
    if (chunk < 8192) chunk = 8192;
    chunk = (chunk + 4095) / 4096 * 4096;
    split = (int)((L + chunk - 1) / chunk);
    hipLaunchKernelGGL(gn_stats4_kernel, dim3(split, x.B * groups), dim3(256), 0, s, x.p, x.sb, x.sc, Cg, groups,
                       L, split, chunk, partials);
  } else {
    hipLaunchKernelGGL(gn_stats_kernel, dim3(split, x.B * groups), dim3(256), 0, s, x.p, x.sb, x.sc, Cg, groups, L,
                       split, partials);
  }
  return split;
}

const float2* gn_mean_rstd(hipStream_t s, const View& x, int groups, double* partials, int given_split) {
  const int split = gn_statistics(s, x, groups, partials, given_split);
  if (split > 64) throw std::invalid_argument("groupnorm: more than 64 statistics slots");
  float2* gst = reinterpret_cast<float2*>(partials + (size_t)x.B * groups * 64 * 2);
  const double n = (double)(x.C / groups) * x.T * x.HW();
  hipLaunchKernelGGL(gn_finalize_kernel, dim3(x.B * groups), dim3(64), 0, s, partials, split, n, gst);
  return gst;
}

}

const float2* groupnorm_affine(hipStream_t s, const View& x, int groups, const float* gamma, const float* beta,
                               double* partials, int given_split) {
  const float2* gst = gn_mean_rstd(s, x, groups, partials, given_split);
  float2* tab = reinterpret_cast<float2*>(partials + (size_t)x.B * groups * 64 * 2 + (size_t)x.B * groups);
  hipLaunchKernelGGL(gn_affine_kernel, dim3(x.B), dim3(256), 0, s, gst, gamma, beta, x.C, x.C / groups, groups, tab);
  return tab;
}

void groupnorm_silu(hipStream_t s, const View& x, const View& out, int groups, const float* gamma,
                    const float* beta, const float* film, int film_row, int film_nt, const int* t_batch,
                    const View* res, double* partials, int given_split) {
  const float2* gst = gn_mean_rstd(s, x, groups, partials, given_split);
  const int Cg = x.C / groups;
  const long L = (long)Cg * x.T * x.HW();
  const bool vec4 = x.HW() % 4 == 0 && L / 4 < (1L << 31) && al16(x.p) && al16(out.p) && x.sb % 4 == 0 &&
                    x.sc % 4 == 0 && out.sb % 4 == 0 && out.sc % 4 == 0 && out.st % 4 == 0 &&
                    (!res || (al16(res->p) && res->sb % 4 == 0 && res->sc % 4 == 0 && res->st % 4 == 0));
  const int HW = x.HW();
  if (vec4 && (long)x.T * HW / 4 >= 1024 && x.st == HW && out.st == HW && (!res || res->st == HW) &&
      (long)x.B * x.C < 65536) {
    const int THW4 = x.T * HW / 4;
// ... 19 lines not shown
                     film_nt, t_batch, res ? res->p : nullptr, res ? res->sb : 0, res ? res->sc : 0,
                     res ? res->st : 0, split2);
}

void groupnorm_silu_x3op(hipStream_t s, const View& x, const X3Op& out, int groups, const float* gamma,
                         const float* beta, const float* film, int film_row, int film_nt, const int* t_batch,
                         double* partials, int given_split) {
  if (x.C % 16 != 0 || out.C != x.C || out.B != x.B || out.T != x.T || out.H != x.H || out.W != x.W)
    throw std::invalid_argument("groupnorm_silu_x3op: operand geometry does not match the input");
  const float2* gst = gn_mean_rstd(s, x, groups, partials, given_split);
  const int Hp = x.H + 2 * out.pad, Wp = x.W + 2 * out.pad;
  const long cg_stride = (long)x.B * x.T * Hp * Wp * 8, hl_stride = (long)(x.C / 16) * cg_stride * 2;
  hipLaunchKernelGGL(gn_apply_x3op_kernel, dim3((x.T * Hp * Wp + 255) / 256, x.B, x.C / 16), dim3(256), 0, s, x.p,
                     x.sb, x.sc, x.st, out.p, cg_stride, hl_stride, x.C, x.C / groups, groups, x.T, x.H, x.W, out.pad,
                     gst, gamma, beta, film, film_row, film_nt, t_batch, x3_range_ptr());
}

void channel_ln(hipStream_t s, const View& out, const View& in0, const View* in1, const float* gamma) {
  const View& i1 = in1 ? *in1 : in0;
  const long npix = (long)out.B * out.T * out.HW();
  auto a16 = [](const void* p) { return ((uintptr_t)p & 15) == 0; };
  auto m4 = [](const View& v) { return v.sb % 4 == 0 && v.sc % 4 == 0 && v.st % 4 == 0; };
  if (out.HW() % 4 == 0 && a16(out.p) && a16(in0.p) && a16(i1.p) && m4(out) && m4(in0) && m4(i1)) {
    hipLaunchKernelGGL(channel_ln4_kernel, dim3((unsigned)((npix / 4 + 31) / 32)), dim3(256), 0, s, out.p, out.sb, out.sc,
                       out.st, in0.p, in0.sb, in0.sc, in0.st, in0.C, i1.p, i1.sb, i1.sc, i1.st, out.C, out.T, out.HW(),
                       out.B, gamma);
    return;
  }
  hipLaunchKernelGGL(channel_ln_kernel, dim3((unsigned)((npix + 31) / 32)), dim3(256), 0, s, out.p, out.sb, out.sc, out.st, in0.p,
                     in0.sb, in0.sc, in0.st, in0.C, i1.p, i1.sb, i1.sc, i1.st, out.C, out.T, out.HW(), out.B, gamma);
}

void temporal_prologue(hipStream_t s, const View& x, const float* gamma, const float* lw, const float* lb,
                       const View& z, const View& r) {
  const long npix = (long)x.B * x.T * x.HW();
  if (npix >= 256L * 1024) {
    hipLaunchKernelGGL(temporal_prologue_kernel, dim3(nblk(npix)), dim3(256), 0, s, x.p, x.sb, x.sc, x.st, x.C, x.T,
                       x.HW(), x.B, gamma, lw, lb, z.p, z.sb, z.sc, z.st, r.p, r.sb, r.sc, r.st);
  } else {
    hipLaunchKernelGGL((temporal_prologue_grp_kernel<16, 16>), dim3((unsigned)((npix + 15) / 16)), dim3(256), 0, s, x.p,
                       x.sb, x.sc, x.st, x.C, x.T, x.HW(), x.B, gamma, lw, lb, z.p, z.sb, z.sc, z.st, r.p, r.sb, r.sc,
                       r.st);
  }
}

void copy_view(hipStream_t s, const View& d, const View& src) {
  const long total = d.numel();
  hipLaunchKernelGGL(copy_kernel, dim3(nblk(total)), dim3(256), 0, s, d.p, d.sb, d.sc, d.st, src.p, src.sb, src.sc,
                     src.st, d.C, d.T, d.HW(), total);
}

void maxpool_hw2(hipStream_t s, const View& d, const View& src) {
  const long total = d.numel();
  hipLaunchKernelGGL(maxpool_kernel, dim3(nblk(total)), dim3(256), 0, s, d.p, d.sb, d.sc, d.st, src.p, src.sb,
                     src.sc, src.st, d.C, d.T, d.H, d.W, src.W, total);
}

void bilinear_frames(hipStream_t s, const View& d, const View& a, const View& b, int t_split) {
  const long total = d.numel();
  if (d.W % 4 == 0 && a.H * a.W <= 1024 && d.T < 65536 && a.H == b.H && a.W == b.W) {
    const int vec = ((uintptr_t)d.p & 15) == 0 && d.sb % 4 == 0 && d.sc % 4 == 0 && d.st % 4 == 0;
    const int nbc = d.B * d.C;
    hipLaunchKernelGGL(bilinear_lds_kernel, dim3((nbc + BPLS - 1) / BPLS, d.T), dim3(256), 0, s, d.p, d.sb, d.sc,
                       d.st, a.p, a.sb, a.sc, a.st, b.p, b.sb, b.sc, b.st, t_split, d.C, nbc, d.H, d.W, a.H, a.W,
                       vec);
    return;
  }
  if (d.W % 4 == 0 && (long)d.B * d.C < 65536 && d.T < 65536) {
    const int vec = ((uintptr_t)d.p & 15) == 0 && d.sb % 4 == 0 && d.sc % 4 == 0 && d.st % 4 == 0;
    const int n4 = d.H * d.W / 4;
    hipLaunchKernelGGL(bilinear4_kernel, dim3((n4 + 255) / 256, d.T, d.B * d.C), dim3(256), 0, s, d.p, d.sb, d.sc,
                       d.st, a.p, a.sb, a.sc, a.st, b.p, b.sb, b.sc, b.st, t_split, d.C, d.H, d.W, a.H, a.W, vec);
    return;
  }
  hipLaunchKernelGGL(bilinear_kernel, dim3(nblk(total)), dim3(256), 0, s, d.p, d.sb, d.sc, d.st, a.p, a.sb, a.sc,
                     a.st, b.p, b.sb, b.sc, b.st, t_split, d.C, d.T, d.H, d.W, a.H, a.W, total);
}

void adaptor_stats(hipStream_t s, const View& x, float* mean, float* std_, double* ) {
  hipLaunchKernelGGL(adaptor_stats_kernel, dim3(x.B * x.C), dim3(256), 0, s, x.p, x.sb, x.sc, x.st, x.C, x.T, x.HW(),
                     mean, std_);
}

void adaptor_normalize(hipStream_t s, const View& d, const View& src, const float* mean, const float* std_) {
  const int bstep = 65535 / d.C;
  for (int b0 = 0; b0 < d.B; b0 += bstep) {
    const int nb = d.B - b0 < bstep ? d.B - b0 : bstep;
    hipLaunchKernelGGL(adaptor_norm_kernel, dim3(nblk((long)d.T * d.HW()), nb * d.C), dim3(256), 0, s,
                       d.p + (long)b0 * d.sb, d.sb, d.sc, d.st, src.p + (long)b0 * src.sb, src.sb, src.sc, src.st,
                       d.C, d.T, d.HW(), mean + (long)b0 * d.C, std_ + (long)b0 * d.C);
  }
}

void zero_pad_frames(hipStream_t s, const View& x) {
  if (!(x.st == (long)x.C * x.HW() && x.sc == x.HW() && x.st % 4 == 0 && x.sb % 4 == 0 &&
        ((uintptr_t)x.p & 15) == 0 && x.B <= 32767 && x.T >= 2))
    throw std::invalid_argument("zero_pad_frames: needs a frame-major buffer of 16-byte aligned frames");
  hipLaunchKernelGGL(zero_pad_frames_kernel, dim3(nblk(x.st / 4), 2 * x.B), dim3(256), 0, s, x.p, x.sb,
                     (long)(x.T - 1) * x.st, x.st / 4);
}

}
```

140-extdm-distribution-extrapolation-diffusion-model-for-video-prediction_amd/csrc/pack.cpp:

```cpp
#include "pack.h"

#include <algorithm>
#include <cmath>

namespace extdm {

template <class T>
int pow2_row_exp(T mx, float& rs) {
  int e = 0;
  if (mx > T(0)) { std::frexp(mx, &e); e = 15 - e; }
  rs = std::ldexp(1.f, -e);
  return e;
}
template int pow2_row_exp<float>(float, float&);
template int pow2_row_exp<double>(double, float&);

void put_hilo(half_t* dst, float v) {
  const half_t hi = (half_t)v;
  dst[0] = hi;
  dst[512] = (_Float16)(v - (float)hi);
}

static half_t* afrag(half_t* blk, int m, int col) { return blk + ((m % 32) + 32 * (col / 8)) * 8 + col % 8; }

// ... 160 lines not shown
            for (int l = 0; l < 64; ++l)
              for (int e = 0; e < 8; ++e) {
                float v;
                if (!elem(mtile, q * 32 + (l & 31), cb, ky, kx, 8 * (l >> 5) + e, v)) continue;
                const size_t base = (((((size_t)mtile * cblks + cb) * 2 + ky) * 2 + kx) * m32 + q) * 2;
                put_hilo(&g[base * 512 + l * 8 + e], v);
              }
  return g;
}

Frags pack_x3_deconv(const fvec& w, int ci, int co, int bm) {
  const int ncb = (ci + 15) / 16, mtc = (co + bm - 1) / bm;
  Frags r{{}, fvec(co), ncb};
  fvec scale(co);
  for (int m = 0; m < co; ++m) {
    float mx = 0.f;
    for (int c = 0; c < ci; ++c)
      for (int tap = 0; tap < 16; ++tap) mx = std::max(mx, std::fabs(w[((size_t)c * co + m) * 16 + tap]));
    scale[m] = std::ldexp(1.f, pow2_row_exp(mx, r.rs[m]));
  }
  r.g = pack_two_tap(4 * mtc, ncb, bm, [&](int mtile, int row, int cb, int ky, int kx, int cc, float& v) {
    const int ph = mtile / mtc, m = (mtile % mtc) * bm + row, c = cb * 16 + cc;
    if (m >= co || c >= ci) return false;
    v = w[(((size_t)c * co + m) * 4 + 3 - (ph >> 1) - 2 * ky) * 4 + 3 - (ph & 1) - 2 * kx] * scale[m];
    return true;
  });
  return r;
}

Frags pack_x3_down(const fvec& w, int co, int ci, int bm) {
  const int ncb = (ci + 15) / 16, mt = (co + bm - 1) / bm;
  Frags r{{}, fvec(co), 4 * ncb};
  fvec scale(co);
  for (int m = 0; m < co; ++m) scale[m] = std::ldexp(1.f, row_exp(&w[(size_t)m * ci * 16], (size_t)ci * 16, r.rs[m]));
  r.g = pack_two_tap(mt, 4 * ncb, bm, [&](int mtile, int row, int cblk, int ky, int kx, int cc, float& v) {
    const int q = cblk / ncb, m = mtile * bm + row, c = (cblk % ncb) * 16 + cc;
    if (m >= co || c >= ci) return false;
    v = w[(((size_t)m * ci + c) * 4 + 2 * ky + 1 - (q >> 1)) * 4 + 2 * kx + 1 - (q & 1)] * scale[m];
    return true;
  });
  return r;
}

HaloPack pack_halo(const fvec& w, int ks, int co, int ci, int bm, int ch) {
  const int kk = ks * ks, cib = 2 * ch, stages = (ci + cib - 1) / cib, mt = (co + bm - 1) / bm;
  const size_t afl = (size_t)ch * kk * 2 * bm;
  HaloPack r{fvec((size_t)mt * stages * afl, 0.f), stages};
  for (int m = 0; m < co; ++m) {
    const int mtile = m / bm, mm = m % bm;
    for (int c = 0; c < ci; ++c) {
      const int st = c / cib, rem = c % cib, half = rem / ch, cp = rem % ch;
      for (int tap = 0; tap < kk; ++tap)
        r.a[((size_t)mtile * stages + st) * afl + ((size_t)(cp * kk + tap) * 2 + half) * bm + mm] = w[((size_t)m * ci + c) * kk + tap];
    }
  }
  return r;
}

fvec pack_narrow(const fvec& w, int kk, int co, int ci, int cot) {
  const int ng = (co + cot - 1) / cot, cotp = (cot + 3) & ~3;
  fvec a((size_t)ng * ci * kk * cotp, 0.f);
  for (int m = 0; m < co; ++m)
    for (int c = 0; c < ci; ++c)
      for (int tap = 0; tap < kk; ++tap)
        a[(((size_t)(m / cot) * ci + c) * kk + tap) * cotp + m % cot] = w[((size_t)m * ci + c) * kk + tap];
  return a;
}

fvec reorder_time3(const fvec& w, int co, int ci, int kt, int kk) {
  fvec r(w.size());
  for (int m = 0; m < co; ++m)
    for (int c = 0; c < ci; ++c)
      for (int z = 0; z < kt; ++z)
        for (int q = 0; q < kk; ++q)
          r[(((size_t)m * kt * ci) + (size_t)z * ci + c) * kk + q] = w[(((size_t)m * ci + c) * kt + z) * kk + q];
  return r;
}

fvec split_channels(const fvec& w, int Co, int Cin, int kk, int lo, int hi) {
  fvec r((size_t)Co * (hi - lo) * kk);
  for (int m = 0; m < Co; ++m)
    std::copy(w.begin() + ((size_t)m * Cin + lo) * kk, w.begin() + ((size_t)m * Cin + hi) * kk,
              r.begin() + (size_t)m * (hi - lo) * kk);
  return r;
}

XPathPack pack_xpath(const fvec& wn, const fvec& bn, const fvec& wi, const fvec& bi, int Cm, int Co, int Cin, int L) {
  const int M32 = (Co + 31) / 32, MP = M32 * 32;
  std::vector<double> V((size_t)Co * 3 * 49 * 49, 0.0), U((size_t)Co * 49, 0.0);
  for (int m = 0; m < Co; ++m)
    for (int ab = 0; ab < 49; ++ab)
      for (int c = 0; c < Cm; ++c) {
        const double wa = wi[((size_t)m * Cin + c) * 49 + ab];
        if (wa == 0.0) continue;
        U[(size_t)m * 49 + ab] += wa * bn[c];
        for (int ci = 0; ci < 3; ++ci) {
          const float* pn = &wn[((size_t)c * 3 + ci) * 49];
          double* pv = &V[(((size_t)m * 3 + ci) * 49 + ab) * 49];
          for (int ef = 0; ef < 49; ++ef) pv[ef] += wa * pn[ef];
        }
      }
  auto valid = [&](int cls1, int a) {
    const int p = cls1 < 3 ? cls1 : (cls1 == 3 ? 3 : L - 7 + cls1), q = p + a - 3;
    return cls1 == 3 || (q >= 0 && q < L);
  };
  const size_t per_cls = (size_t)3 * 13 * M32 * 1024;
  XPathPack r{std::vector<half_t>(49 * per_cls), fvec((size_t)49 * MP), fvec((size_t)49 * MP)};
  std::vector<double> K((size_t)Co * 3 * 169);
  for (int cls = 0; cls < 49; ++cls) {
    const int cy = cls / 7, cx = cls % 7;
    std::fill(K.begin(), K.end(), 0.0);
    for (int m = 0; m < Co; ++m) {
      double cbv = bi[m];
      for (int a = 0; a < 7; ++a)
        for (int b = 0; b < 7; ++b) {
          if (!valid(cy, a) || !valid(cx, b)) continue;
          cbv += U[(size_t)m * 49 + a * 7 + b];
          for (int ci = 0; ci < 3; ++ci) {
            const double* pv = &V[(((size_t)m * 3 + ci) * 49 + a * 7 + b) * 49];
            double* pk = &K[((size_t)m * 3 + ci) * 169];
            for (int e = 0; e < 7; ++e)
              for (int f = 0; f < 7; ++f) pk[(a + e) * 13 + (b + f)] += pv[e * 7 + f];
          }
        }
      r.cb[(size_t)cls * MP + m] = (float)cbv;
      const int e2 = row_exp(&K[(size_t)m * 3 * 169], 3 * 169, r.rs[(size_t)cls * MP + m]);
      for (int ci = 0; ci < 3; ++ci)
        for (int dy = 0; dy < 13; ++dy)
          for (int dx = 0; dx < 13; ++dx) {
            const float v = (float)std::ldexp(K[((size_t)m * 3 + ci) * 169 + dy * 13 + dx], e2);
            put_hilo(afrag(&r.g[(size_t)cls * per_cls + ((size_t)(ci * 13 + dy) * M32 + m / 32) * 1024], m, dx), v);
          }
    }
  }
  return r;
}

Frags pack_conv7c3(const fvec& w, int Cm) {
  const int M32 = (Cm + 31) / 32;
  Frags r{std::vector<half_t>((size_t)12 * M32 * 1024), fvec(M32 * 32, 0.f)};
  for (int m = 0; m < Cm; ++m) {
    const int e2 = row_exp(&w[(size_t)m * 147], 147, r.rs[m]);
    for (int ci = 0; ci < 3; ++ci)
      for (int dy = 0; dy < 7; ++dy)
        for (int dx = 0; dx < 7; ++dx) {
          const float v = std::ldexp(w[(((size_t)m * 3 + ci) * 7 + dy) * 7 + dx], e2);
          put_hilo(afrag(&r.g[((size_t)(ci * 4 + dy / 2) * M32 + m / 32) * 1024], m, 8 * (dy % 2) + dx), v);
        }
  }
  return r;
}

static double up_true(int r, int k, int n) {
  if (r < 0 || r >= 2 * n) return 0.0;
  const double src = std::max(0.0, (r + 0.5) * 0.5 - 0.5);
  const int k0 = (int)src, k1 = k0 < n - 1 ? k0 + 1 : k0;
  const double lam = src - k0;
  return (k == k0 ? 1.0 - lam : 0.0) + (k == k1 ? lam : 0.0);
}
static double up_inf(int r, int k) {
  const int j = (r >= 0 ? r : r - 1) / 2;
  if (k == j) return 0.75;
  return (r - 2 * j == 0 ? k == j - 1 : k == j + 1) ? 0.25 : 0.0;
}

FeaPhasePack pack_fea_phase(const fvec& wt, int Co, int Cf, int n) {
// ... 173 lines not shown
```

140-extdm-distribution-extrapolation-diffusion-model-for-video-prediction_amd/csrc/pack.h:

```cpp
#pragma once
#include <algorithm>
#include <cmath>
#include <cstddef>
#include <vector>

namespace extdm {

using half_t = _Float16;
using fvec = std::vector<float>;

template <class T>
int pow2_row_exp(T mx, float& rs);
void put_hilo(half_t* dst, float v);

struct Frags {
  std::vector<half_t> g;
  fvec rs;
  int n = 0;
  std::vector<half_t> tap_major;
};
template <class F>
Frags pack_frags(int npar, int M, int K, int bm, F&& elem) {
  const int nkt = (K + 31) / 32, mt = (M + bm - 1) / bm, m32 = bm / 32;
  const size_t ah = (size_t)2 * m32 * 2 * 512;
  Frags r{std::vector<half_t>((size_t)npar * mt * nkt * ah), fvec(M), nkt};
  fvec scale(M);
  for (int m = 0; m < M; ++m) {
    float mx = 0.f, v;
    for (int par = 0; par < npar; ++par)
      for (int k = 0; k < K; ++k)
        if (elem(par, m, k, v)) mx = std::max(mx, std::fabs(v));
    scale[m] = std::ldexp(1.f, pow2_row_exp(mx, r.rs[m]));
  }
  for (int par = 0; par < npar; ++par)
    for (int mtile = 0; mtile < mt; ++mtile)
      for (int kt = 0; kt < nkt; ++kt)
        for (int st = 0; st < 2; ++st)
          for (int q = 0; q < m32; ++q)
            for (int l = 0; l < 64; ++l)
              for (int e = 0; e < 8; ++e) {
                const int m = mtile * bm + q * 32 + (l & 31), k = kt * 32 + st * 16 + 8 * (l >> 5) + e;
                float v;
                if (m >= M || k >= K || !elem(par, m, k, v)) continue;
                const size_t base = (((size_t)par * mt + mtile) * nkt + kt) * ah + (size_t)((st * m32 + q) * 2) * 512;
                put_hilo(&r.g[base + l * 8 + e], v * scale[m]);
              }
  return r;
}

struct GemmPlane { fvec a; int Mpad = 0, Kpad = 0; };
GemmPlane pack_gemm_plane(const fvec& w, int M, int K, int bm);
GemmPlane pack_deconv_planes(const fvec& w, int ci, int co, int bm);
Frags pack_gemm_x3(const GemmPlane& p, int npar, int M, int K, int bm, int kk);
Frags pack_unit3d(const fvec& w, int M, int Cin, int Cpad, int KS, int bm, int stem_row);
Frags pack_conv2d(const fvec& w, int M, int Cin, int Cpad, int KS, int bm, int stem_row);
struct TilesF32 { fvec a; int nkt = 0; };
TilesF32 pack_conv3d_f32(const fvec& w, int M, int Cin, int Cpad, int KS, int bm);
TilesF32 pack_conv3d_f32_stem(const fvec& w, int M, int Cin, int KS, int bm, int stem_row);
Frags pack_x3(const fvec& w, int ks, int co, int ci, int bm, int ng);
Frags pack_x3_deconv(const fvec& w, int ci, int co, int bm);
Frags pack_x3_down(const fvec& w, int co, int ci, int bm);
struct HaloPack { fvec a; int stages = 0; };
HaloPack pack_halo(const fvec& w, int ks, int co, int ci, int bm, int ch);
fvec pack_narrow(const fvec& w, int kk, int co, int ci, int cot);
fvec reorder_time3(const fvec& w, int co, int ci, int kt, int kk);
fvec split_channels(const fvec& w, int Co, int Cin, int kk, int lo, int hi);

struct XPathPack { std::vector<half_t> g; fvec rs, cb; };
XPathPack pack_xpath(const fvec& wn, const fvec& bn, const fvec& wi, const fvec& bi, int Cm, int Co, int Cin, int L);
Frags pack_conv7c3(const fvec& w, int Cm);
struct FeaPhasePack { fvec k5, side_scale, corner; std::vector<half_t> side; };
FeaPhasePack pack_fea_phase(const fvec& wt, int Co, int Cf, int n);

fvec pack_stw_rows(const fvec& w, int nmat, int rows, int K);
struct AttnX3Pack { std::vector<half_t> a; float sc[5] = {}, s2 = 1.f; };
AttnX3Pack pack_attn_x3(const fvec& wqkv, const fvec& wproj, const fvec& ng, const fvec* nb, int C, int hid, int uh,
                        float q_scale);

struct Affine { fvec a, b; };
Affine bn_fold_f32(const fvec& w, const fvec& b, const fvec& rm, const fvec& rv);
Affine bn_fold_f64(const fvec& w, const fvec& b, const fvec& rm, const fvec& rv);

}
```

140-extdm-distribution-extrapolation-diffusion-model-for-video-prediction_amd/csrc/runtime.cpp:

```cpp
#include <hip/hip_runtime.h>

#include <algorithm>
#include <functional>
#include <cmath>
#include <cstdarg>
#include <cstdio>
#include <cstring>
#include <memory>
#include <stdexcept>
#include <string>
#include <unordered_map>
#include <vector>

#include "extdm.h"
#include "host_util.h"
#include "kernels.h"
#include "pack.h"

using namespace extdm;

static constexpr int kTrajHeads = 8;

namespace {

// ... 528 lines not shown
      for (int i = 0; i < 64; ++i)
        for (int j = 0; j < 64; ++j)
          t[((size_t)hd * 64 + i) * 64 + j] = j >= g.D ? -INFINITY : time_bias_host[((size_t)hd * 64 + i) * 64 + j] * s2;
    float* d = upload(t);
    mask_bias[key] = {d, 1};
    return d;
  }

  float* packed_stw(const std::string& n, int nmat) {
    const std::string key = n + (nmat == 3 ? "#stwqkv" : "#stwproj");
    auto it = dev.find(key);
    if (it != dev.end()) return it->second;
    const HostTensor& t = H(n);
    REQUIRE(nmat == 1 || (int)t.shape[0] == 3 * cfg.heads * cfg.dim_head, "qkv weight rows != 3 * heads * dim_head: " + n);
    return dev[key] = upload(pack_stw_rows(t.f, nmat, (int)t.shape[0] / nmat, (int)t.shape[1]));
  }
  struct AttnX3W { void* w = nullptr; float* sc = nullptr; float s2 = 1.f; };
  std::unordered_map<std::string, AttnX3W> attn_x3w;
  const AttnX3W& packed_attn_x3(const std::string& nqkv, const std::string& nproj, const std::string& ng,
                                const std::string& nb) {
    auto it = attn_x3w.find(nqkv);
    if (it != attn_x3w.end()) return it->second;
    const HostTensor& tq = H(nqkv);
    const HostTensor& tp = H(nproj);
    const HostTensor& tg = H(ng);
    const int C = (int)tq.shape[1], hid = cfg.heads * cfg.dim_head, uh = attn_x3_unit_halves(C);
    REQUIRE((int)tq.shape[0] == 3 * hid && (int)tp.shape[0] == C && (int)tp.shape[1] == hid,
            "attention weight shapes: " + nqkv);
    REQUIRE(uh > 0, "attention x3 layout: unsupported channel count");
    REQUIRE((int)tg.f.size() == C, "attention norm affine size: " + ng);
    const AttnX3Pack a = pack_attn_x3(tq.f, tp.f, tg.f, nb.empty() ? nullptr : &H(nb).f, C, hid, uh, q_scale());
    return attn_x3w[nqkv] = {upload(a.a), upload(std::vector<float>(a.sc, a.sc + 5)), a.s2};
  }
  bool x3_convs() const { return cfg.precision == EXTDM_PRECISION_F16X3 || cfg.precision == EXTDM_PRECISION_BF16_ATTN; }
  bool bf16_attn() const { return cfg.precision == EXTDM_PRECISION_BF16_ATTN; }
  bool x3_attn_ok(int C, int ntok, int mode) const {
    const bool off = env_flag("EXTDM_NO_X3_ATTN"), off_stw = env_flag("EXTDM_NO_X3_STW"), off_tmp = env_flag("EXTDM_NO_X3_TEMPORAL");
    if (off || (mode == 0 && off_stw) || (mode == 1 && off_tmp)) return false;
    return (cfg.precision == EXTDM_PRECISION_F16X3 || (bf16_attn() && cfg.dim_head == 32)) &&
           attn_x3_supported(C, ntok, cfg.dim_head, cfg.heads);
  }
  bool stw64_ok(int C, int ntok) const {
    static const bool off = env_flag("EXTDM_NO_STW64");
    return !off && x3_convs() && stw64_x3_supported(C, ntok, cfg.dim_head, cfg.heads);
  }
  bool fused_ok(int C, int ntok) const {
    static const bool off = env_flag("EXTDM_NO_FUSED_STW");
    return !off && fused_attn_supported(C, ntok, cfg.dim_head, cfg.heads);
  }
  bool core_attn(int ntok, int max_tok, bool fused_x3, bool window) const {
    if (!(cfg.dim_head == 32 || (cfg.dim_head == 16 && window && !bf16_attn())) || ntok > max_tok) return false;
    if (bf16_attn()) return !fused_x3;
    static const bool off = env_flag("EXTDM_NO_X3_CORE");
    return cfg.precision == EXTDM_PRECISION_F16X3 && !fused_x3 && !off;
  }
  float q_scale() const { return 1.0f / std::sqrt((float)cfg.dim_head); }
  int tm() const { return cfg.arch == EXTDM_ARCH_WO_REF ? cfg.tc - 1 : cfg.tc; }
  int frames() const { return tm() + cfg.tp; }

  int bench_stage = 0;
  bool last_core = false;
  std::unordered_map<int, std::string> bench_kernel;

  void stw(const std::string& p, const View& x, bool shifted) {
    const AttnGeom g = stw_geom(x.T, x.H, x.W, shifted);
    const int N = g.ws0 * g.ws1 * g.ws2;
    const int bstride = cfg.window[0] * cfg.window[1] * cfg.window[2] <= 32 ? 32 : 64;
    const bool fused_x3 = bstride == 32 && x3_attn_ok(x.C, N, 0);
    if (bstride == 64 && stw64_ok(x.C, N)) {
      const std::string a = p + ".fn.fn.attn";
      const AttnX3W& w = packed_attn_x3(a + ".qkv.weight", a + ".proj.weight", p + ".fn.norm.gamma", "");
      int npat = 1;
      const float* mb = stw_mask_bias64(p, g, npat, w.s2);
      if (plan) return;
      REQUIRE(stw64_x3(s, x, g, cfg.heads, cfg.dim_head, D(p + ".fn.norm.gamma"), w.w, w.sc, D(a + ".proj.bias"), mb,
                       npat, rope_cos, rope_sin, q_scale(), bf16_attn()),
              "f16x3 64-token STW launch rejected");
      return;
    }
    if (core_attn(N, 64, fused_x3, true)) {
      last_core = true;
      Scope sc(arena);
      const int hid = cfg.heads * cfg.dim_head;
      View ln = alloc_cf(x.B, x.C, x.T, x.H, x.W);
      if (!plan && bench_stage == 0) channel_ln(s, ln, x, nullptr, D(p + ".fn.norm.gamma"));
      View qkv = alloc_cf(x.B, 3 * hid, x.T, x.H, x.W);
      if (bench_stage == 0 || bench_stage == 2) conv(qkv, ln, nullptr, P(p + ".fn.fn.attn.qkv.weight"), 1, 0, nullptr);
      View o = alloc_cf(x.B, hid, x.T, x.H, x.W);
      if (!plan && (bench_stage == 0 || bench_stage == 1))
        REQUIRE(attention_core(s, qkv, o, g, cfg.heads, cfg.dim_head, bias_dense.at(p), bstride, rope_cos, rope_sin,
                               q_scale(), bf16_attn()),
                "STW attention core launch rejected");
      if (bench_stage == 0 || bench_stage == 3)
        conv(x, o, nullptr, P(p + ".fn.fn.attn.proj.weight"), 1, 0, D(p + ".fn.fn.attn.proj.bias"), &x);
      return;
    }
    if (fused_x3) {
      const std::string a = p + ".fn.fn.attn";
      const AttnX3W& w = packed_attn_x3(a + ".qkv.weight", a + ".proj.weight", p + ".fn.norm.gamma", "");
      int npat = 1;
      const float* mb = stw_mask_bias(p, g, npat, w.s2);
      if (plan) return;
      REQUIRE(stw_x3(s, x, g, cfg.heads, cfg.dim_head, D(p + ".fn.norm.gamma"), w.w, w.sc, D(a + ".proj.bias"),
                     mb, npat, rope_cos, rope_sin, q_scale(), bf16_attn()),
              "f16x3 STW launch rejected");
      return;
    }
    if (fused_ok(x.C, N)) {
      const std::string a = p + ".fn.fn.attn";
      float* wq = packed_stw(a + ".qkv.weight", 3);
      float* wp = packed_stw(a + ".proj.weight", 1);
      if (plan) return;
      REQUIRE(stw_fused(s, x, g, cfg.heads, cfg.dim_head, D(p + ".fn.norm.gamma"), wq, wp, D(a + ".proj.bias"),
                        bias_dense.at(p), bstride, rope_cos, rope_sin, q_scale()),
              "fused STW launch rejected");
      return;
    }
    REQUIRE(cfg.dim_head == 32 && N <= 32 && bstride == 32, "STW attention shape without a kernel (C=" + std::to_string(x.C) +
                                               ", window tokens " + std::to_string(N) + ")");
    Scope sc(arena);
    const int hid = cfg.heads * 32;
    View ln = alloc_cf(x.B, x.C, x.T, x.H, x.W);
    if (!plan) channel_ln(s, ln, x, nullptr, D(p + ".fn.norm.gamma"));
    View qkv = alloc_cf(x.B, 3 * hid, x.T, x.H, x.W);
    conv(qkv, ln, nullptr, P(p + ".fn.fn.attn.qkv.weight"), 1, 0, nullptr);
    View o = alloc_cf(x.B, hid, x.T, x.H, x.W);
    if (!plan) window_attention(s, qkv, o, g, cfg.heads, bias_dense.at(p), rope_cos, rope_sin, q_scale());
    conv(x, o, nullptr, P(p + ".fn.fn.attn.proj.weight"), 1, 0, D(p + ".fn.fn.attn.proj.bias"), &x);
  }

  void temporal_long(const std::string& p, const View& x, const View& out, AttnGeom g) {
    const std::string a = p + ".fn.fn.fn";
    const int T = x.T;
    REQUIRE(T <= 64 && tb_stride == 64, "temporal attention over more than 64 frames");
    g.per = 64;
    const bool x3 = cfg.precision == EXTDM_PRECISION_F16X3 || (bf16_attn() && cfg.dim_head == 32);
    if (x3 && !env_flag("EXTDM_NO_T64") && !env_flag("EXTDM_NO_X3_ATTN") && !env_flag("EXTDM_NO_X3_TEMPORAL") &&
        temporal64_x3_supported(x.C, T, cfg.dim_head, cfg.heads) && out.sb == x.sb && out.sc == x.sc && out.st == x.st &&
        x.st == (long)x.H * x.W && ((long)(x.C - 1) * x.sc + (long)T * x.st) * 4 < (1L << 30)) {
      const AttnX3W& w = packed_attn_x3(a + ".attn.to_qkv.weight", a + ".attn.to_out.weight", a + ".norm.weight",
                                        a + ".norm.bias");
      const float* mb = temporal_mask_bias64(g, w.s2);
      if (plan) return;
      REQUIRE(temporal64_x3(s, x, out, g, cfg.heads, cfg.dim_head, D(p + ".fn.norm.gamma"), D(a + ".norm.weight"),
                            D(a + ".norm.bias"), w.w, w.sc, mb, rope_cos, rope_sin, q_scale(), bf16_attn()),
              "f16x3 64-slot temporal attention launch rejected");
      return;
    }
    static const bool off = env_flag("EXTDM_NO_X3_CORE");
    const bool core = bf16_attn() ? cfg.dim_head == 32 : (cfg.precision == EXTDM_PRECISION_F16X3 && !off);
    last_core = core;
    Scope sc(arena);
    const int hid = cfg.heads * cfg.dim_head;
    View z = alloc_cf(x.B, x.C, T, x.H, x.W), rr = alloc_cf(x.B, x.C, T, x.H, x.W);
    if (!plan && bench_stage == 0)
      temporal_prologue(s, x, D(p + ".fn.norm.gamma"), D(a + ".norm.weight"), D(a + ".norm.bias"), z, rr);
    View qkv = alloc_cf(x.B, 3 * hid, T, x.H, x.W);
    if (bench_stage == 0 || bench_stage == 2) conv(qkv, z, nullptr, P(a + ".attn.to_qkv.weight"), 1, 0, nullptr);
    View o = alloc_cf(x.B, hid, T, x.H, x.W);
    if (!plan && (bench_stage == 0 || bench_stage == 1)) {
      if (core)
        REQUIRE(attention_core(s, qkv, o, g, cfg.heads, cfg.dim_head, time_bias, 64, rope_cos, rope_sin, q_scale(),
                               bf16_attn()),
                "64-slot temporal attention core launch rejected");
      else
        REQUIRE(temporal_attention64(s, qkv, o, g, cfg.heads, cfg.dim_head, time_bias, rope_cos, rope_sin, q_scale()),
                "fp32 64-frame temporal attention launch rejected");
    }
    if (bench_stage == 0 || bench_stage == 3) conv(out, o, nullptr, P(a + ".attn.to_out.weight"), 1, 0, nullptr, &rr);
  }

  void temporal(const std::string& p, const View& x, const View& out) {
    const std::string a = p + ".fn.fn.fn";
    const int T = x.T;
    AttnGeom g{};
    g.mode = 1; g.D = T; g.H = x.H; g.W = x.W;
    static const bool per8 = [] { const char* v = getenv("EXTDM_X3_PER8"); return !(v && v[0] == '0'); }();
    g.per = T <= 8 && per8 ? 8 : (T <= 16 ? 16 : 32);
    if (T > 32) { temporal_long(p, x, out, g); return; }
    const bool fused_x3 = x3_attn_ok(x.C, T, 1) && out.sc == x.sc && out.st == x.st;
    if (core_attn(T, 32, fused_x3, false)) {
      last_core = true;
      Scope sc(arena);
      const int hid = cfg.heads * 32;
      View z = alloc_cf(x.B, x.C, T, x.H, x.W), rr = alloc_cf(x.B, x.C, T, x.H, x.W);
      if (!plan && bench_stage == 0)
        temporal_prologue(s, x, D(p + ".fn.norm.gamma"), D(a + ".norm.weight"), D(a + ".norm.bias"), z, rr);
      View qkv = alloc_cf(x.B, 3 * hid, T, x.H, x.W);
      if (bench_stage == 0 || bench_stage == 2) conv(qkv, z, nullptr, P(a + ".attn.to_qkv.weight"), 1, 0, nullptr);
      View o = alloc_cf(x.B, hid, T, x.H, x.W);
      if (!plan && (bench_stage == 0 || bench_stage == 1))
        REQUIRE(attention_core(s, qkv, o, g, cfg.heads, cfg.dim_head, time_bias, 32, rope_cos, rope_sin, q_scale(),
                               bf16_attn()),
                "temporal attention core launch rejected");
      if (bench_stage == 0 || bench_stage == 3) conv(out, o, nullptr, P(a + ".attn.to_out.weight"), 1, 0, nullptr, &rr);
      return;
    }
    if (fused_x3) {
      const AttnX3W& w = packed_attn_x3(a + ".attn.to_qkv.weight", a + ".attn.to_out.weight", a + ".norm.weight",
                                        a + ".norm.bias");
      const float* mb = temporal_mask_bias(g, w.s2);
      if (plan) return;
      REQUIRE(temporal_x3(s, x, out, g, cfg.heads, cfg.dim_head, D(p + ".fn.norm.gamma"), D(a + ".norm.weight"),
                          D(a + ".norm.bias"), w.w, w.sc, mb,
                          rope_cos, rope_sin, q_scale(), bf16_attn()),
              "f16x3 temporal attention launch rejected");
      return;
    }
    if (fused_ok(x.C, T) && T <= 32) {
      float* wq = packed_stw(a + ".attn.to_qkv.weight", 3);
      float* wo = packed_stw(a + ".attn.to_out.weight", 1);
      if (plan) return;
      REQUIRE(temporal_fused(s, x, out, g, cfg.heads, cfg.dim_head, D(p + ".fn.norm.gamma"), D(a + ".norm.weight"),
                             D(a + ".norm.bias"), wq, wo, time_bias, 32, rope_cos, rope_sin, q_scale()),
              "fused temporal attention launch rejected");
      return;
    }
    REQUIRE(cfg.dim_head == 32 && T <= 32, "temporal attention shape without a kernel");
    Scope sc(arena);
    const int hid = cfg.heads * 32;
    View z = alloc_cf(x.B, x.C, T, x.H, x.W), rr = alloc_cf(x.B, x.C, T, x.H, x.W);
    if (!plan) temporal_prologue(s, x, D(p + ".fn.norm.gamma"), D(a + ".norm.weight"), D(a + ".norm.bias"), z, rr);
    View qkv = alloc_cf(x.B, 3 * hid, T, x.H, x.W);
    conv(qkv, z, nullptr, P(a + ".attn.to_qkv.weight"), 1, 0, nullptr);
    View o = alloc_cf(x.B, hid, T, x.H, x.W);
    if (!plan) window_attention(s, qkv, o, g, cfg.heads, time_bias, rope_cos, rope_sin, q_scale());
    conv(out, o, nullptr, P(a + ".attn.to_out.weight"), 1, 0, nullptr, &rr);
  }

  AdaptorGeom adaptor_geom() const {
    const int L = std::max(1, (int)std::ceil(std::log2((double)(cfg.tp + 1) / tm())));
    return {L, ((1 << L) - 1) * tm()};
  }

  void adaptor(const std::string& p, const View& x) {
    Scope sc(arena);
    const int B = x.B, C = x.C, Hh = x.H, Ww = x.W, tc = tm(), tp = cfg.tp, HW = Hh * Ww;
    const AdaptorGeom ag = adaptor_geom();
    const std::string ap = p + ".adaptors";
    View E = alloc_tm(B, C, tc << ag.L, Hh, Ww);
    {
      Scope s2(arena);
      View ln = alloc_cf(B, C, tc, Hh, Ww);
      View xm = x.frames(0, tc);
      if (!plan) channel_ln(s, ln, xm, nullptr, D(ap + ".predictor.fn.norm.gamma"));
      conv(E.frames(0, tc), ln, nullptr, P(ap + ".predictor.fn.fn.weight"), 1, 0, D(ap + ".predictor.fn.fn.bias"),
           &xm);
    }
    for (int l = 0; l < ag.L; ++l) {
      Scope s2(arena);
      const int nl = tc << l;
      const std::string wn = ap + ".extrapolators." + std::to_string(l) + ".fn.weight";
      const bool t3 = H(wn).shape[2] == 3;
      float* mean = arena.alloc((size_t)B * C);
      float* sd = arena.alloc((size_t)B * C);
      View cur = E.frames(0, nl);
      if (!plan) adaptor_stats(s, cur, mean, sd, partials);
      if (!t3) {
        View hn = alloc_tm(B, C, nl, Hh, Ww);
        if (!plan) adaptor_normalize(s, hn, cur, mean, sd);
        conv(E.frames(nl, nl), hn, nullptr, P(wn), 1, 1, nullptr, &hn, ACT_NONE, sd, mean);
      } else {
        View hp = alloc_tm(B, C, nl + 2, Hh, Ww);
        View hn = hp.frames(1, nl);
        if (!plan) {
          zero_pad_frames(s, hp);
          adaptor_normalize(s, hn, cur, mean, sd);
        }
        View win = hp;
        win.C = 3 * C; win.T = nl;
        conv(E.frames(nl, nl), win, nullptr, Ptime3(wn), 1, 1, nullptr, &hn, ACT_NONE, sd, mean);
      }
    }
    View ein = E.frames(tc, ag.F);
    ein.C = ag.F * C; ein.T = 1; ein.sc = HW; ein.st = 0;
    View mo = alloc_tm(B, C, tp, Hh, Ww);
    View mo2 = mo;
    mo2.C = tp * C; mo2.T = 1; mo2.sc = HW; mo2.st = 0;
    conv(mo2, ein, nullptr, P(p + ".Tmodulator.weight"), 1, 0, D(p + ".Tmodulator.bias"));
    View xp = x.frames(tc, tp);
    View lnf = alloc_cf(B, 2 * C, tp, Hh, Ww);
    if (!plan) channel_ln(s, lnf, mo, &xp, D(p + ".fuser.norm.gamma"));
    conv(xp, lnf, nullptr, P(p + ".fuser.fn.weight"), 1, 0, D(p + ".fuser.fn.bias"), &xp);
  }

  void trajwarp_kv(const View& fea) {
    const std::string c = "init_traj.cross_att";
    View fm = fea.frames(0, cfg.tc);
    conv(with_batch(kv_k, fea.B), fm, nullptr, P(c + ".linear_k.weight"), 1, 0, D(c + ".linear_k.bias"), nullptr,
         ACT_RELU);
    conv(with_batch(kv_v, fea.B), fm, nullptr, P(c + ".linear_v.weight"), 1, 0, D(c + ".linear_v.bias"), nullptr,
         ACT_RELU);
    if (!plan && kv_split_ok())
      REQUIRE(cross_kv_split(s, kv_k.p, kv_v.p, kvp, fea.B, fea.C, kTrajHeads, cfg.tc * cfg.fea_size * cfg.fea_size),
              "TrajWarp: k / v split not covered");
  }
  bool kv_split_ok() const {
    static const bool staged = env_flag("EXTDM_CROSS_STAGED");
    static const bool off = env_flag("EXTDM_NO_X3_CROSS");
    return kvp != nullptr && !staged && !off && x3_convs() && cfg.fea_ch == 32 * kTrajHeads;
  }
  void trajwarp_q(const View& xq, const View& fea, const View& fp_out) {
    Scope sc(arena);
    const int B = xq.B, C = fea.C, tc = cfg.tc, tp = cfg.tp, fs = cfg.fea_size;
    REQUIRE(xq.H == fs && xq.W == fs, "TrajWarp: maxpooled latent must match cond_fea size");
    const std::string c = "init_traj.cross_att";
    View q = alloc_cf(B, C, tp, fs, fs);
    conv(q, xq, nullptr, P(c + ".linear_q.weight"), 1, 0, D(c + ".linear_q.bias"), nullptr, ACT_RELU);
    View a = alloc_cf(B, C, tp, fs, fs);
    if (!plan) {
      static const bool off = env_flag("EXTDM_NO_X3_CROSS");
      const bool x3 = !off && x3_convs() &&
                      (kv_split_ok() ? cross_attention_x3p(s, q.p, kvp, a.p, B, C, kTrajHeads, tp * fs * fs, tc * fs * fs)
                                     : cross_attention_x3(s, q.p, kv_k.p, kv_v.p, a.p, B, C, kTrajHeads, tp * fs * fs,
                                                          tc * fs * fs));
      if (!x3) cross_attention(s, q.p, kv_k.p, kv_v.p, a.p, B, C, kTrajHeads, tp * fs * fs, tc * fs * fs);
    }
    View fm2p = alloc_cf(B, C, tp, fs, fs);
    conv(fm2p, a, nullptr, P(c + ".linear_o.weight"), 1, 0, D(c + ".linear_o.bias"), nullptr, ACT_RELU);
    View fp = fea.frames(tc, tp);
    conv(fp_out, fp, &fm2p, P("init_traj.fuser.weight"), 1, 0, D("init_traj.fuser.bias"));
  }

  View r_all, kv_k, kv_v, fup_all, fa_all;
  View fr_all;
  _Float16* kvp = nullptr;
  void alloc_cond_cache() {
    const int Bm = cfg.max_batch, T = frames(), L = cfg.latent, fs = cfg.fea_size;
    r_all = cf_view(dmalloc((size_t)Bm * cfg.dim * T * L * L * 4), Bm, cfg.dim, T, L, L);
    if (cfg.arch == EXTDM_ARCH_U12) {
      kv_k = cf_view(dmalloc((size_t)Bm * cfg.fea_ch * cfg.tc * fs * fs * 4), Bm, cfg.fea_ch, cfg.tc, fs, fs);
      kv_v = cf_view(dmalloc((size_t)Bm * cfg.fea_ch * cfg.tc * fs * fs * 4), Bm, cfg.fea_ch, cfg.tc, fs, fs);
      if (cfg.fea_ch == 32 * kTrajHeads)
        kvp = reinterpret_cast<_Float16*>(
            dmalloc(cross_kv_halves(Bm, cfg.fea_ch, kTrajHeads, cfg.tc * fs * fs) * sizeof(_Float16)));
    }
    if (cfg.arch == EXTDM_ARCH_ADA || cfg.arch == EXTDM_ARCH_ADA_U22)
      fup_all = cf_view(dmalloc((size_t)Bm * cfg.fea_ch * T * L * L * 4), Bm, cfg.fea_ch, T, L, L);
    if (cfg.arch == EXTDM_ARCH_ADA && fea_phase_on())
      fa_all = cf_view(dmalloc((size_t)Bm * cfg.fea_ch * T * fs * fs * 4), Bm, cfg.fea_ch, T, fs, fs);
    if (fea_hoist_on())
      fr_all = cf_view(dmalloc((size_t)Bm * cfg.dim * cfg.tp * L * L * 4), Bm, cfg.dim, cfg.tp, L, L);
  }
  static View with_batch(View v, int B) { v.B = B; return v; }

  void prepare_cond(int B, const float* cond, const float* fea) {
    Scope top(arena);
    const int arch = cfg.arch;
    const int tc = tm(), T = frames(), L = cfg.latent, fs = cfg.fea_size;
    View vc = cf_view(const_cast<float*>(cond), B, 3, cfg.tc, L, L);
    View vf = cf_view(const_cast<float*>(fea), B, cfg.fea_ch, T, fs, fs);
    View r = with_batch(r_all, B).frames(0, tc);
    if (arch == EXTDM_ARCH_WO_REF) {
      REQUIRE(fs == L, "wo_ref: cond_fea must be at the latent resolution");
      const View fc = vf.frames(0, tc);
      init_conv_cond(r, vc.frames(0, tc), fc);
      hoist_fea(B, vf.frames(tc, cfg.tp));
      return;
    }
    View fup;
    if (arch == EXTDM_ARCH_U12) {
      trajwarp_kv(vf);
      fup = alloc_cf(B, cfg.fea_ch, tc, L, L);
      if (!plan) bilinear_frames(s, fup, vf.frames(0, tc), vf.frames(0, tc), tc);
    } else {
      View fa = fa_all.p ? with_batch(fa_all, B) : alloc_cf(B, cfg.fea_ch, T, fs, fs);
// ... 1223 lines not shown
      HIPCHK(hipEventRecord(e0, s));
      for (int i = 0; i < iters; ++i) launch();
      HIPCHK(hipEventRecord(e1, s));
      HIPCHK(hipEventSynchronize(e1));
      float ms = 0.f;
      HIPCHK(hipEventElapsedTime(&ms, e0, e1));
      (void)hipEventDestroy(e0);
      (void)hipEventDestroy(e1);
      *ms_out = ms / iters;
      *flops_out = flop;
      return;
    }
    REQUIRE(layer != 11, "bench layer 11: the phase-composed cond_fea branch is off");
    if (layer == 12 || layer == 13) {
      std::string wn = layer == 12 ? "init_traj.cross_att.linear_q.weight" : "downs.2.4.Tmodulator.weight";
      REQUIRE(h->has(wn), "bench layer weight missing: " + wn);
      const PackedW& w = h->P(wn);
      const std::string bn = wn.substr(0, wn.size() - 6) + "bias";
      View in, out;
      double flop = 0;
      if (layer == 12) {
        const int fs = h->cfg.fea_size, C = (int)h->H(wn).shape[0];
        in = h->alloc_cf(B, C, h->cfg.tp, fs, fs);
        out = h->alloc_cf(B, C, h->cfg.tp, fs, fs);
        flop = 2.0 * B * h->cfg.tp * fs * fs * (double)C * C;
      } else {
        const int Ls = L >> 2, K = (int)h->H(wn).shape[1], M = (int)h->H(wn).shape[0];
        in = h->alloc_tm(B, K, 1, Ls, Ls);
        out = h->alloc_tm(B, M, 1, Ls, Ls);
        in.st = 0; out.st = 0;
        flop = 2.0 * B * Ls * Ls * (double)K * M;
      }
      fill_normal(s, in.p, 1, (int)in.numel(), 17, 0, 0, 7);
      auto launch = [&, in, out] { h->conv(out, in, nullptr, w, 1, 0, h->D(bn), nullptr, layer == 12 ? ACT_RELU : ACT_NONE); };
      note_kernel("");
      launch();
      h->bench_kernel[layer] = noted_kernel();
      hipEvent_t e0, e1;
      HIPCHK(hipEventCreate(&e0));
      HIPCHK(hipEventCreate(&e1));
      HIPCHK(hipEventRecord(e0, s));
      for (int i = 0; i < iters; ++i) launch();
      HIPCHK(hipEventRecord(e1, s));
      HIPCHK(hipEventSynchronize(e1));
      float ms = 0.f;
      HIPCHK(hipEventElapsedTime(&ms, e0, e1));
      (void)hipEventDestroy(e0);
      (void)hipEventDestroy(e1);
      *ms_out = ms / iters;
      *flops_out = flop;
      return;
    }
    if (layer == 18 || layer == 19) {
      const bool upl = layer == 18;
      const std::string ix = h->cfg.arch == EXTDM_ARCH_ADA_U22 ? ".6" : ".5";
      const std::string pre = upl ? "ups." + std::to_string(h->cfg.n_levels - 2) + ix : "downs.0" + ix;
      REQUIRE(h->cfg.n_levels >= 2 && h->has(pre + ".weight"), "bench layer weight missing: " + pre + ".weight");
      const auto& sh = h->H(pre + ".weight").shape;
      const int c_in = (int)sh[upl ? 0 : 1], c_out = (int)sh[upl ? 1 : 0];
      const int Li = upl ? L / 2 : L, Lo = upl ? L : L / 2;
      View in = h->alloc_cf(B, c_in, T, Li, Li), out = h->alloc_cf(B, c_out, T, Lo, Lo);
      fill_normal(s, in.p, 1, (int)in.numel(), 17, 0, 0, 1);
      const PackedW& w = upl ? h->Pdeconv(pre + ".weight") : h->P(pre + ".weight");
      float* bias = h->D(pre + ".bias");
      auto launch = [&, in, out] { h->conv(out, in, nullptr, w, upl ? 1 : 2, upl ? 0 : 1, bias); };
      note_kernel("");
      launch();
      h->bench_kernel[layer] = noted_kernel();
      hipEvent_t e0, e1;
      HIPCHK(hipEventCreate(&e0));
      HIPCHK(hipEventCreate(&e1));
      HIPCHK(hipEventRecord(e0, s));
      for (int i = 0; i < iters; ++i) launch();
      HIPCHK(hipEventRecord(e1, s));
      HIPCHK(hipEventSynchronize(e1));
      float ms = 0.f;
      HIPCHK(hipEventElapsedTime(&ms, e0, e1));
      (void)hipEventDestroy(e0);
      (void)hipEventDestroy(e1);
      *ms_out = ms / iters;
      *flops_out = 2.0 * B * T * (double)(upl ? Li : Lo) * (upl ? Li : Lo) * (double)c_out * c_in * 16;
      return;
    }
    static const char* names[] = {"init_conv.weight", "downs.0.0.block2.proj.weight", "downs.1.0.block2.proj.weight",
                                  "downs.2.0.block2.proj.weight", "ups.3.0.res_conv.weight",
                                  "downs.0.0.block2.proj.weight"};
    static const int levels[] = {0, 0, 1, 2, 0, 0};
    REQUIRE(layer >= 0 && layer < 6, "unknown layer id");
    std::string wn = names[layer];
    const bool fea_only = layer == 0 && h->xpath_enabled();
    if (fea_only) {
      h->Pxpath();
      wn = "init_conv.weight#fea";
    }
    REQUIRE(h->has(wn), "bench layer weight missing: " + wn);
    const auto& sh = h->H(wn).shape;
    const int co = (int)sh[0], ci = (int)sh[1], ks = (int)sh.back();
    const int Lq = L >> levels[layer];
    const int c1 = layer == 0 && !fea_only ? h->cfg.fea_ch : 0, c0 = ci - c1;
    View x0 = h->alloc_cf(B, c0, T, Lq, Lq);
    View fup = c1 ? h->alloc_cf(B, c1, T, Lq, Lq) : x0;
    View r = h->alloc_cf(B, co, T, Lq, Lq);
    fill_normal(s, x0.p, 1, (int)x0.numel(), 17, 0, 0, 1);
    if (c1) fill_normal(s, fup.p, 1, (int)fup.numel(), 17, 0, 0, 2);
    const PackedW& w = h->P(wn);
    const std::string bn = wn.substr(0, wn.size() - 6) + "bias";
    float* bias = h->has(bn) ? h->D(bn) : nullptr;
    const View* in1 = c1 ? &fup : nullptr;
    X3Op op;
    if (layer == 5) {
      REQUIRE(h->x3_convs() && conv_x3_op_supported(r, w, c0, 1),
              "bench layer 5: the operand-input conv is not covered (f16x3 only)");
      op.B = B; op.C = c0; op.T = T; op.H = Lq; op.W = Lq; op.pad = 1;
      op.p = reinterpret_cast<_Float16*>(h->arena.alloc((x3op_halves(B, c0, T, Lq, Lq, 1) + 1) / 2));
      groupnorm_silu_x3op(s, x0, op, 8, h->D("downs.0.0.block1.norm.weight"), h->D("downs.0.0.block1.norm.bias"),
                          nullptr, 0, 0, nullptr, h->partials, 0);
    }
    auto launch = [&] {
      if (layer == 5) {
        ConvEpi e;
        e.bias = bias;
        REQUIRE(conv_x3_forward_op(s, r, op, w, e), "bench layer 5: launch not covered");
      } else {
        h->conv(r, x0, in1, w, 1, ks / 2, bias);
      }
    };
    note_kernel("");
    launch();
    h->bench_kernel[layer] = noted_kernel();
    hipEvent_t a, b;
    HIPCHK(hipEventCreate(&a));
    HIPCHK(hipEventCreate(&b));
    HIPCHK(hipEventRecord(a, s));
    for (int i = 0; i < iters; ++i) launch();
    HIPCHK(hipEventRecord(b, s));
    HIPCHK(hipEventSynchronize(b));
    float ms = 0.f;
    HIPCHK(hipEventElapsedTime(&ms, a, b));
    (void)hipEventDestroy(a);
    (void)hipEventDestroy(b);
    *ms_out = ms / iters;
    *flops_out = 2.0 * B * T * Lq * Lq * (double)co * ci * ks * ks;
  });
}

int extdm_bench_layer_kernel(ExtdmHandle* h, int layer, char* buf, int cap) {
  return guarded([&] {
    REQUIRE(h && buf && cap > 0, "bench_layer_kernel: arguments");
    auto it = h->bench_kernel.find(layer);
    const std::string v = it == h->bench_kernel.end() ? std::string() : it->second;
    std::snprintf(buf, (size_t)cap, "%s", v.c_str());
  });
}

int extdm_decode(ExtdmHandle* h, int B, int C, int T, int S, int fh, int fw, const float* ref, const float* flow,
                 const float* occ, float* pred, float* warped, void* stream) {
  return guarded([&] {
    REQUIRE(h, "null handle");
    HIPCHK(hipSetDevice(h->cfg.device));
    h->s = reinterpret_cast<hipStream_t>(stream);
    if (occ) {
      REQUIRE(h->finalized, "handle not finalized");
      REQUIRE(B <= h->cfg.max_batch && T <= h->cfg.tc + h->cfg.tp, "decode exceeds the planned batch");
      REQUIRE(C == h->cfg.num_channels && S == h->cfg.image, "decode geometry differs from the config");
    }
    h->decode(B, T, S, fh, fw, ref, flow, occ, pred, warped);
// ... 67 lines not shown
```

Measured before the change: 36.61 frames/s.

## Fold adaptor normalization and channel LayerNorm into conv input staging

Adds an input-affine mode to the split-f16 conv kernel. Mode 1 applies per-sample per-channel adaptor mean/std normalization from an LDS table while staging X. Mode 2 applies per-pixel channel-LN mean/rstd to 1x1 fuser convs. The separate normalize/LN passes and their intermediate tensors are replaced by lightweight stats kernels, which cuts memory traffic and launches. The cost is extra LDS for the table, more template instantiations, and reordered post-scale/residual epilogue math that could slightly change numerics.

After: 37.83 frames/s, median of 6. 3.3% higher.

```diff
diff --git a/140-extdm-distribution-extrapolation-diffusion-model-for-video-prediction_amd/csrc/conv_x3.hip b/140-extdm-distribution-extrapolation-diffusion-model-for-video-prediction_amd/csrc/conv_x3.hip
--- a/140-extdm-distribution-extrapolation-diffusion-model-for-video-prediction_amd/csrc/conv_x3.hip
+++ b/140-extdm-distribution-extrapolation-diffusion-model-for-video-prediction_amd/csrc/conv_x3.hip
@@ -40,6 +40,7 @@
   int mtc;
   int in0_bytes, in1_bytes;
   ConvEpi e;
+  int aff_ns;
 };
 
 __device__ __forceinline__ float act_apply(float v, int act) {
@@ -84,7 +85,7 @@
 template <> struct XMaxX3<5, 256> { static constexpr int v = 400; };
 
 template <int KS, int KY, int BM, int BN, int NG, int WN, int NW, int XBUF, bool SPAN, int NS, bool XOP = false,
-          bool RGN = false, int SPL = 0, bool PH = false, bool WS = false, bool BX = false, int TT = 0>
+          bool RGN = false, int SPL = 0, bool PH = false, bool WS = false, bool BX = false, int TT = 0, int AFF = 0>
 __global__ __launch_bounds__(NW * 64) __attribute__((amdgpu_waves_per_eu(NW == 4 && KS == 5 ? 2 : 1))) void conv_x3_kernel(X3Args a) {
   constexpr int NT = NW * 64;
   constexpr int PAD = KS / 2;
@@ -103,6 +104,8 @@
   constexpr int TN = BN / (32 * WN);
   static_assert(TM >= 1 && TN >= 1 && WM * WN == NW, "bad tile");
   static_assert(!XOP || (NG == 1 && XBUF == 2 && SPAN), "operand input: one group, two X buffers");
+  static_assert(!AFF || (SPAN && BX && !XOP && !WS && !PH && TT == 0 && (AFF == 2 ? SPL != 2 : NG == 1)),
+                "AFF: buffer-load staging (SPL = 2 with AFF = 1: the epilogue order alone)");
 
   extern __shared__ __attribute__((aligned(16))) _Float16 smx[];
   static_assert(!WS || (NG == 1 && SPAN && SPL != 2 && NW % 2 == 0), "WS: one group, spanning barriers");
@@ -150,10 +153,13 @@
   };
 
   int sg[NSLOT], spos[NSLOT], soff0[NSLOT], soff1[NSLOT];
+  int arow[NSLOT];
+  float2 amr[NSLOT];
 #pragma unroll
   for (int j = 0; j < NSLOT; ++j) {
     const int sl = tid + NT * j;
     sg[j] = -1; spos[j] = 0; soff0[j] = -1; soff1[j] = -1;
+    arow[j] = -1; amr[j] = make_float2(0.f, 0.f);
     if (sl < a.XPOS * NG) {
       const int g = sl / a.XPOS, pos = sl - g * a.XPOS;
       const int p = pos / (THK * a.RS);
@@ -167,6 +173,8 @@
         const int ip = TT == 2 ? 4 * iy * a.W + 2 * ix : iy * a.W + ix;
         soff0[j] = (int)((long)b * a.i0b + (long)t * a.i0t) + ip;
         soff1[j] = (int)((long)b * a.i1b + (long)t * a.i1t) + ip;
+        if (AFF == 1) arow[j] = (b - plane0 / a.T) * a.Cin * 2;
+        if (AFF == 2) amr[j] = a.e.in_aff[(long)q * (a.H * a.W) + ip];
       }
     }
   }
@@ -264,6 +272,8 @@
     }
   };
   _Float16* const xdummy = Xs0 + XB * XH + (WSR ? 2 * 16 * RP : 0);
+  float* const atab = reinterpret_cast<float*>(xdummy + 32) + 2 * BM;
+  float* const azero = atab + a.aff_ns * a.Cin * 2;
   auto store_x = [&](_Float16* Xs, int cgb) __attribute__((always_inline)) {
 #pragma unroll
     for (int j = 0; j < NSLOT; ++j) {
@@ -277,6 +287,19 @@
           if (!bufx) r *= xmask(j, cgb, c);
         }
         v[c] = r;
+      }
+      if (AFF == 1) {
+        const float* tp = arow[j] >= 0 ? atab + arow[j] + cgb * (2 * CIB) : azero;
+#pragma unroll
+        for (int c = 0; c < 16; c += 2) {
+          const float4 mr = *reinterpret_cast<const float4*>(tp + 2 * c);
+          v[c] = (v[c] - mr.x) * mr.y;
+          v[c + 1] = (v[c + 1] - mr.z) * mr.w;
+        }
+      }
+      if (AFF == 2) {
+#pragma unroll
+        for (int c = 0; c < 16; ++c) v[c] = (v[c] - amr[j].x) * amr[j].y;
       }
       unsigned hw[8], lw[8];
       float am = 0.f;
@@ -418,6 +441,14 @@
     const int mc = m < a.Cout ? m : a.Cout - 1;
     ep_sc[tid] = a.wscale[mc];
     ep_bi[tid] = a.e.bias ? a.e.bias[mc] : 0.f;
+  }
+  if (AFF == 1 && SPL != 2) {
+    const int bf = plane0 / a.T, nb = a.P / a.T;
+    float2* const at2 = reinterpret_cast<float2*>(atab);
+    for (int i = tid; i < a.aff_ns * a.Cin; i += NT)
+      at2[i] = bf + i / a.Cin < nb ? a.e.in_aff[(long)bf * a.Cin + i] : make_float2(0.f, 0.f);
+    if (tid < 16) at2[a.aff_ns * a.Cin + tid] = make_float2(0.f, 0.f);
+    __syncthreads();
   }
   if (SPL == 2) {
     const long per = (long)TM * TN * 16 * NT;
@@ -639,6 +670,13 @@
       float v[16];
 #pragma unroll
       for (int r16 = 0; r16 < 16; ++r16) v[r16] = acc[i][j][r16] * scl[r16] + bia[r16];
+      if (AFF == 1 && has_post) {
+        float ps[16];
+#pragma unroll
+        for (int r16 = 0; r16 < 16; ++r16) ps[r16] = a.e.post_scale[post_pc ? mrow[r16] : b * a.Cout + mrow[r16]];
+#pragma unroll
+        for (int r16 = 0; r16 < 16; ++r16) v[r16] = v[r16] * ps[r16];
+      }
       if (has_res) {
         const int rbase = (int)((long)b * a.e.res_sb + (long)t * a.e.res_st) + pix;
         float rv[16];
@@ -657,7 +695,7 @@
 #pragma unroll
         for (int r16 = 0; r16 < 16; ++r16) v[r16] += rv[r16];
       }
-      if (has_post) {
+      if (AFF != 1 && has_post) {
         float ps[16], pt[16];
 #pragma unroll
         for (int r16 = 0; r16 < 16; ++r16) {
@@ -842,13 +880,13 @@
   return v3;
 }
 
-bool x3_w128_4(const X3Args& a, bool xop) {
+bool x3_w128_4(const X3Args& a, bool xop, size_t extra_halves = 0) {
   static const int w = [] { const char* v = getenv("EXTDM_X3_W128"); return v ? atoi(v) : 4; }();
   if (w == 8) return false;
   constexpr size_t AH = 3 * 4 * 2 * 512;
   const size_t xlo = xop ? (size_t)((a.XPOS + 63) & ~63) * 16
                          : (EXTDM_X3_LIN == 1 ? (size_t)((a.XPOS + 1 + 63) & ~63) * 16 : (size_t)a.XPOS * 16);
-  return (2 * AH + 2 * 2 * xlo + 32 + 4 * 128) * sizeof(_Float16) <= 80 * 1024;
+  return (2 * AH + 2 * 2 * xlo + 32 + 4 * 128 + extra_halves) * sizeof(_Float16) <= 80 * 1024;
 }
 void x3_split128(bool four, long& max_wg, long& max_total) {
   static const long* t4 = [] {
@@ -977,8 +1015,130 @@
   return nwg >= 192;
 }
 
+namespace {
+
+template <int KS, int BM, int BN, int NG, int WN, int NW, int NS, int SPL, int AFF>
+void launch_aff(hipStream_t s, const X3Args& a, unsigned ntiles, size_t lds) {
+  const auto kern = &conv_x3_kernel<KS, 1, BM, BN, NG, WN, NW, 2, true, NS, false, false, SPL, false, false, true, 0, AFF>;
+  static bool attr = false;
+  if (!attr) {
+    (void)hipFuncSetAttribute(reinterpret_cast<const void*>(kern), hipFuncAttributeMaxDynamicSharedMemorySize, 160 * 1024);
+    attr = true;
+  }
+  note_kernel("conv_x3_kernel<%d, 1, %d, %d, %d, %d, %d, 2, true, %d, false, false, %d, false, false, true, 0, %d>", KS, BM,
+              BN, NG, WN, NW, NS, SPL, AFF);
+  hipLaunchKernelGGL(kern, dim3(ntiles, (a.Cout + BM - 1) / BM, SPL == 1 ? a.nsplit : 1), dim3(NW * 64), lds, s, a);
+}
+
+bool x3_aff_setup(const View& out, const View& in0, const View* in1, const PackedW& w, const ConvEpi& epi, int mode,
+                  X3Args& a, unsigned& ntiles, size_t* lds, int* split) {
+  if (out.p == in0.p || (in1 && out.p == in1->p)) {
+    if (mode != 2 || out.C > w.xbm || out.sb != (out.p == in0.p ? in0.sb : in1->sb)) return false;
+  }
+  static const bool nospan = env_flag("EXTDM_X3_NOSPAN");
+  if (nospan || EXTDM_X3_LIN == 1 || (mode != 1 && mode != 2)) return false;
+  if (!x3_setup(out, in0, in1, w, epi, a, ntiles, nullptr) || a.e.stats) return false;
+  const int ks = w.KH, bm = w.xbm, bn = w.xbn, ng = w.xng;
+  if (!x3_bufx_ok(a, 16 * ng) || epi.res_aff) return false;
+  size_t tab = 0;
+  *split = 0;
+  if (mode == 1) {
+    if (ks != 3 || ng != 1 || in1 || x3_v3() == 1 || x3_ws(kWsStaged64)) return false;
+    a.aff_ns = a.T % a.NP == 0 ? 1 : (a.NP % a.T == 0 ? a.NP / a.T : (a.NP + a.T - 2) / a.T + 1);
+    tab = ((size_t)a.aff_ns * a.Cin + 16) * 4;
+    if (bm == 64 && bn == 256) {
+      if ((a.XPOS + 255) / 256 > 3) return false;
+    } else if (bm == 128 && bn == 128) {
+      long mw, mt;
+      x3_split128(true, mw, mt);
+      if (!x3_w128_4(a, false, tab)) return false;
+      *split = split_slices(a, ntiles, mw, mt);
+    } else {
+      return false;
+    }
+  } else {
+    if (ks != 1 || ng != 2 || a.XPOS > bn) return false;
+    if (bm == 256 && bn == 128) *split = x3_split256() ? split_slices(a, ntiles, 256, 256, 256) : 0;
+    else if (bm == 128 && bn == 128) *split = split_slices(a, ntiles, 384, 512);
+    else if (!((bm == 64 && bn == 128) || (bm == 256 && bn == 256))) return false;
+  }
+  const size_t AH = (size_t)ng * ks * (bm / 32) * 2 * 512;
+  const size_t lds0 = (2 * AH + 2 * 2 * (size_t)a.XPOS * ng * 16 + 32 + 4 * bm) * sizeof(_Float16);
+  *lds = lds0 + tab * sizeof(_Float16);
+  return *lds <= 160 * 1024 && (160 * 1024) / *lds == (160 * 1024) / lds0;
+}
+
+bool conv_x3_forward_aff(hipStream_t s, const View& out, const View& in0, const View* in1, const PackedW& w,
+                         const ConvEpi& epi) {
+  X3Args a;
+  unsigned ntiles = 0;
+  size_t lds = 0;
+  int S = 0;
+  const int mode = epi.in_aff_mode;
+  if (!epi.in_aff || !x3_aff_setup(out, in0, in1, w, epi, mode, a, ntiles, &lds, &S)) return false;
+  if (mode == 1) {
+    if (!epi.post_first || !epi.post_scale || !epi.res) return false;
+    const int need = (a.XPOS + 255) / 256;
+    if (w.xbm == 64) {
+      if (need <= 1) launch_aff<3, 64, 256, 1, 4, 4, 1, 0, 1>(s, a, ntiles, lds);
+      else if (need == 2) launch_aff<3, 64, 256, 1, 4, 4, 2, 0, 1>(s, a, ntiles, lds);
+      else launch_aff<3, 64, 256, 1, 4, 4, 3, 0, 1>(s, a, ntiles, lds);
+    } else if (S) {
+      if (!epi.split_ws || split_bytes(a, ntiles, S) > epi.split_ws_bytes) return false;
+      a.part = epi.split_ws;
+      a.nsplit = S;
+      if (need <= 1) launch_aff<3, 128, 128, 1, 2, 4, 1, 1, 1>(s, a, ntiles, lds);
+      else launch_aff<3, 128, 128, 1, 2, 4, 2, 1, 1>(s, a, ntiles, lds);
+      launch_aff<3, 128, 128, 1, 2, 4, 1, 2, 1>(s, a, ntiles, lds);
+    } else {
+      if (need <= 1) launch_aff<3, 128, 128, 1, 2, 4, 1, 0, 1>(s, a, ntiles, lds);
+      else launch_aff<3, 128, 128, 1, 2, 4, 2, 0, 1>(s, a, ntiles, lds);
+    }
+    return true;
+  }
+  if (epi.post_first) return false;
+  a.mfast = x3_mfast(a, X3Tile{w.xbm, w.xbn, w.xng}, ntiles);
+  if (S) {
+    if (!epi.split_ws || split_bytes(a, ntiles, S) > epi.split_ws_bytes) return false;
+    a.part = epi.split_ws;
+    a.nsplit = S;
+    if (w.xbm == 256) {
+      launch_aff<1, 256, 128, 2, 2, 8, 1, 1, 2>(s, a, ntiles, lds);
+      launch_sp<1, 1, 256, 128, 2, 2, 8, 2, true, 1, false, false, 2>(s, a, ntiles);
+    } else {
+      launch_aff<1, 128, 128, 2, 2, 4, 1, 1, 2>(s, a, ntiles, lds);
+      launch_sp<1, 1, 128, 128, 2, 2, 4, 2, true, 1, false, false, 2>(s, a, ntiles);
+    }
+    return true;
+  }
+  if (w.xbm == 64) launch_aff<1, 64, 128, 2, 4, 4, 1, 0, 2>(s, a, ntiles, lds);
+  else if (w.xbm == 128) launch_aff<1, 128, 128, 2, 2, 4, 1, 0, 2>(s, a, ntiles, lds);
+  else if (w.xbn == 256) launch_aff<1, 256, 256, 2, 2, 8, 1, 0, 2>(s, a, ntiles, lds);
+  else launch_aff<1, 256, 128, 2, 2, 8, 1, 0, 2>(s, a, ntiles, lds);
+  return true;
+}
+
+}
+
+bool conv_x3_aff_covers(const View& out, const View& in0, const View* in1, const PackedW& w0, int mode) {
+  if (!w0.wx || w0.mode != MODE_CONV || w0.KH != w0.KW) return false;
+  PackedW wt = w0;
+  if (x3_bn256(out, w0, ConvEpi{})) wt.xbn = 256;
+  X3Args a;
+  unsigned ntiles = 0;
+  size_t lds = 0;
+  int S = 0;
+  return x3_aff_setup(out, in0, in1, wt, ConvEpi{}, mode, a, ntiles, &lds, &S);
+}
+
 bool conv_x3_forward(hipStream_t s, const View& out, const View& in0, const View* in1, const PackedW& w0,
                      const ConvEpi& epi, int* stats_slots) {
+  if (epi.in_aff_mode) {
+    if (stats_slots) *stats_slots = 0;
+    PackedW wa = w0;
+    if (x3_bn256(out, w0, epi)) wa.xbn = 256;
+    return conv_x3_forward_aff(s, out, in0, in1, wa, epi);
+  }
   PackedW wt = w0;
   if (x3_bn256(out, w0, epi)) wt.xbn = 256;
   const PackedW& w = wt;
diff --git a/140-extdm-distribution-extrapolation-diffusion-model-for-video-prediction_amd/csrc/kernels.h b/140-extdm-distribution-extrapolation-diffusion-model-for-video-prediction_amd/csrc/kernels.h
--- a/140-extdm-distribution-extrapolation-diffusion-model-for-video-prediction_amd/csrc/kernels.h
+++ b/140-extdm-distribution-extrapolation-diffusion-model-for-video-prediction_amd/csrc/kernels.h
@@ -121,6 +121,9 @@
   const float2* res_aff = nullptr;
   float* split_ws = nullptr;
   size_t split_ws_bytes = 0;
+  int in_aff_mode = 0;
+  const float2* in_aff = nullptr;
+  int post_first = 0;
 };
 
 int halo_ch(int ks, int bm);
@@ -133,6 +136,7 @@
 bool conv_x3_forward(hipStream_t s, const View& out, const View& in0, const View* in1, const PackedW& w,
                      const ConvEpi& epi, int* stats_slots = nullptr);
 bool conv_x3_covers(const View& out, const View& in0, const View* in1, const PackedW& w);
+bool conv_x3_aff_covers(const View& out, const View& in0, const View* in1, const PackedW& w, int mode);
 size_t conv_x3_split_bytes(const View& out, const View& in0, const View* in1, const PackedW& w);
 size_t conv_x3_op_split_bytes(const View& out, const PackedW& w, int C);
 struct X3Op {
@@ -273,6 +277,8 @@
 void bilinear_frames(hipStream_t s, const View& dst, const View& a, const View& b, int t_split);
 void adaptor_stats(hipStream_t s, const View& x, float* mean, float* std_, double* partials);
 void adaptor_normalize(hipStream_t s, const View& dst, const View& src, const float* mean, const float* std_);
+void adaptor_stats_inc(hipStream_t s, const View& x, long n_prev, double2* carry, float2* mr, float* std_);
+void channel_ln_stats(hipStream_t s, float2* out, const View& in0, const View* in1);
 void zero_pad_frames(hipStream_t s, const View& x);
 
 struct StepCoef {
diff --git a/140-extdm-distribution-extrapolation-diffusion-model-for-video-prediction_amd/csrc/norm.hip b/140-extdm-distribution-extrapolation-diffusion-model-for-video-prediction_amd/csrc/norm.hip
--- a/140-extdm-distribution-extrapolation-diffusion-model-for-video-prediction_amd/csrc/norm.hip
+++ b/140-extdm-distribution-extrapolation-diffusion-model-for-video-prediction_amd/csrc/norm.hip
@@ -397,6 +397,81 @@
   }
 }
 
+__global__ __launch_bounds__(256) void channel_ln_stats4_kernel(float2* out, const float* p0, long sb0, long sc0,
+                                                                long st0, int C0, const float* p1, long sb1,
+                                                                long sc1, long st1, int C, int T, int HW, int B) {
+  __shared__ double red[8][32][4], red2[8][32][4];
+  const int q = threadIdx.x & 31, grp = threadIdx.x >> 5;
+  const long nq = (long)B * T * HW / 4;
+  const long idx = (long)blockIdx.x * 32 + q;
+  const bool ok = idx < nq;
+  const long pix = (ok ? idx : 0) * 4;
+  const int hw = (int)(pix % HW);
+  const int t = (int)((pix / HW) % T);
+  const int b = (int)(pix / ((long)HW * T));
+  const long b0 = (long)b * sb0 + (long)t * st0 + hw;
+  const long b1 = (long)b * sb1 + (long)t * st1 + hw;
+  double s[4] = {0.0, 0.0, 0.0, 0.0}, ss[4] = {0.0, 0.0, 0.0, 0.0};
+  if (ok) {
+#pragma unroll 4
+    for (int c = grp; c < C; c += 8) {
+      const float4 v = c < C0 ? *reinterpret_cast<const float4*>(p0 + b0 + (long)c * sc0)
+                              : *reinterpret_cast<const float4*>(p1 + b1 + (long)(c - C0) * sc1);
+      const double d[4] = {v.x, v.y, v.z, v.w};
+#pragma unroll
+      for (int k = 0; k < 4; ++k) { s[k] += d[k]; ss[k] += d[k] * d[k]; }
+    }
+  }
+#pragma unroll
+  for (int k = 0; k < 4; ++k) { red[grp][q][k] = s[k]; red2[grp][q][k] = ss[k]; }
+  __syncthreads();
+  if (threadIdx.x < 128) {
+    const int qq = threadIdx.x >> 2, k = threadIdx.x & 3;
+    const long px = ((long)blockIdx.x * 32 + qq) * 4 + k;
+    double tt = 0.0, t2 = 0.0;
+    for (int i = 0; i < 8; ++i) { tt += red[i][qq][k]; t2 += red2[i][qq][k]; }
+    const double mean = tt / C;
+    double var = t2 / C - mean * mean;
+    if (var < 0) var = 0;
+    if (px < nq * 4) out[px] = make_float2((float)mean, 1.f / sqrtf((float)var + 1e-5f));
+  }
+}
+
+__global__ __launch_bounds__(256) void channel_ln_stats_kernel(float2* out, const float* p0, long sb0, long sc0,
+                                                               long st0, int C0, const float* p1, long sb1,
+                                                               long sc1, long st1, int C, int T, int HW, int B) {
+  __shared__ double red[8][33], red2[8][33];
+  const int px = threadIdx.x & 31, grp = threadIdx.x >> 5;
+  const long idx = (long)blockIdx.x * 32 + px;
+  const long npix = (long)B * T * HW;
+  const bool ok = idx < npix;
+  const long id2 = ok ? idx : 0;
+  const int hw = (int)(id2 % HW);
+  const int t = (int)((id2 / HW) % T);
+  const int b = (int)(id2 / ((long)HW * T));
+  const long b0 = (long)b * sb0 + (long)t * st0 + hw;
+  const long b1 = (long)b * sb1 + (long)t * st1 + hw;
+  double s = 0.0, ss = 0.0;
+  if (ok)
+    for (int c = grp; c < C; c += 8) {
+      const double v = ld2(p0, b0, sc0, C0, p1, b1, sc1, c);
+      s += v;
+      ss += v * v;
+    }
+  red[grp][px] = s;
+  red2[grp][px] = ss;
+  __syncthreads();
+  if (threadIdx.x < 32) {
+    const long o = (long)blockIdx.x * 32 + threadIdx.x;
+    double tt = 0.0, t2 = 0.0;
+    for (int i = 0; i < 8; ++i) { tt += red[i][threadIdx.x]; t2 += red2[i][threadIdx.x]; }
+    const double mean = tt / C;
+    double var = t2 / C - mean * mean;
+    if (var < 0) var = 0;
+    if (o < npix) out[o] = make_float2((float)mean, 1.f / sqrtf((float)var + 1e-5f));
+  }
+}
+
 __global__ __launch_bounds__(256) void channel_ln_kernel(float* out, long osb, long osc, long ost,
                                                          const float* p0, long sb0, long sc0, long st0, int C0,
                                                          const float* p1, long sb1, long sc1, long st1, int C,
@@ -721,6 +796,44 @@
   }
 }
 
+__global__ __launch_bounds__(256) void adaptor_stats_inc_kernel(const float* x, long sb, long sc, long st, int C, int T,
+                                                                int HW, long n_prev, double2* carry, float2* mr,
+                                                                float* std_out) {
+  const int bc = blockIdx.x;
+  const int b = bc / C, c = bc % C;
+  const float* p = x + (long)b * sb + (long)c * sc;
+  const int n = T * HW;
+  const double k = p[0];
+  double s = 0.0, q = 0.0;
+  int t = threadIdx.x / HW, hw = threadIdx.x - t * HW;
+  const int dt = 256 / HW, dhw = 256 - dt * HW;
+  for (int e = threadIdx.x; e < n; e += 256) {
+    const double d = p[(long)t * st + hw] - k;
+    s += d;
+    q += d * d;
+    t += dt; hw += dhw;
+    if (hw >= HW) { hw -= HW; ++t; }
+  }
+  __shared__ double sh[8];
+  block_sum2(s, q, sh);
+  if (threadIdx.x == 0) {
+    double mean = k + s / n, m2 = q - s * s / n;
+    if (m2 < 0) m2 = 0;
+    long cnt = n;
+    if (n_prev > 0) {
+      const double2 a = carry[bc];
+      const double na = (double)n_prev, nb = (double)n, delta = mean - a.x;
+      cnt = n_prev + n;
+      mean = a.x + delta * nb / (na + nb);
+      m2 = a.y + m2 + delta * delta * na * nb / (na + nb);
+    }
+    carry[bc] = make_double2(mean, m2);
+    const float sd = sqrtf((float)(m2 / (double)(cnt - 1)) + 1e-5f);
+    mr[bc] = make_float2((float)mean, 1.f / sd);
+    std_out[bc] = sd;
+  }
+}
+
 __global__ __launch_bounds__(256) void adaptor_norm_kernel(float* d, long dsb, long dsc, long dst_, const float* s,
                                                            long ssb, long ssc, long sst, int C, int T, int HW,
                                                            const float* mean, const float* std_) {
@@ -906,6 +1019,26 @@
                      mean, std_);
 }
 
+void adaptor_stats_inc(hipStream_t s, const View& x, long n_prev, double2* carry, float2* mr, float* std_) {
+  hipLaunchKernelGGL(adaptor_stats_inc_kernel, dim3(x.B * x.C), dim3(256), 0, s, x.p, x.sb, x.sc, x.st, x.C, x.T,
+                     x.HW(), n_prev, carry, mr, std_);
+}
+
+void channel_ln_stats(hipStream_t s, float2* out, const View& in0, const View* in1) {
+  const View& i1 = in1 ? *in1 : in0;
+  const int C = in0.C + (in1 ? in1->C : 0);
+  const long npix = (long)in0.B * in0.T * in0.HW();
+  auto a16 = [](const void* p) { return ((uintptr_t)p & 15) == 0; };
+  auto m4 = [](const View& v) { return v.sb % 4 == 0 && v.sc % 4 == 0 && v.st % 4 == 0; };
+  if (in0.HW() % 4 == 0 && a16(in0.p) && a16(i1.p) && m4(in0) && m4(i1)) {
+    hipLaunchKernelGGL(channel_ln_stats4_kernel, dim3((unsigned)((npix / 4 + 31) / 32)), dim3(256), 0, s, out, in0.p,
+                       in0.sb, in0.sc, in0.st, in0.C, i1.p, i1.sb, i1.sc, i1.st, C, in0.T, in0.HW(), in0.B);
+    return;
+  }
+  hipLaunchKernelGGL(channel_ln_stats_kernel, dim3((unsigned)((npix + 31) / 32)), dim3(256), 0, s, out, in0.p, in0.sb,
+                     in0.sc, in0.st, in0.C, i1.p, i1.sb, i1.sc, i1.st, C, in0.T, in0.HW(), in0.B);
+}
+
 void adaptor_normalize(hipStream_t s, const View& d, const View& src, const float* mean, const float* std_) {
   const int bstep = 65535 / d.C;
   for (int b0 = 0; b0 < d.B; b0 += bstep) {
diff --git a/140-extdm-distribution-extrapolation-diffusion-model-for-video-prediction_amd/csrc/pack.cpp b/140-extdm-distribution-extrapolation-diffusion-model-for-video-prediction_amd/csrc/pack.cpp
--- a/140-extdm-distribution-extrapolation-diffusion-model-for-video-prediction_amd/csrc/pack.cpp
+++ b/140-extdm-distribution-extrapolation-diffusion-model-for-video-prediction_amd/csrc/pack.cpp
@@ -266,6 +266,14 @@
   for (int m = 0; m < Co; ++m)
     std::copy(w.begin() + ((size_t)m * Cin + lo) * kk, w.begin() + ((size_t)m * Cin + hi) * kk,
               r.begin() + (size_t)m * (hi - lo) * kk);
+  return r;
+}
+
+fvec fold_ln_gamma(const fvec& w, const fvec& gamma, int Co, int Cin) {
+  fvec r((size_t)Co * Cin);
+  for (int m = 0; m < Co; ++m)
+    for (int c = 0; c < Cin; ++c)
+      r[(size_t)m * Cin + c] = (float)((double)w[(size_t)m * Cin + c] * (double)gamma[c]);
   return r;
 }
 
diff --git a/140-extdm-distribution-extrapolation-diffusion-model-for-video-prediction_amd/csrc/pack.h b/140-extdm-distribution-extrapolation-diffusion-model-for-video-prediction_amd/csrc/pack.h
--- a/140-extdm-distribution-extrapolation-diffusion-model-for-video-prediction_amd/csrc/pack.h
+++ b/140-extdm-distribution-extrapolation-diffusion-model-for-video-prediction_amd/csrc/pack.h
@@ -65,6 +65,7 @@
 fvec pack_narrow(const fvec& w, int kk, int co, int ci, int cot);
 fvec reorder_time3(const fvec& w, int co, int ci, int kt, int kk);
 fvec split_channels(const fvec& w, int Co, int Cin, int kk, int lo, int hi);
+fvec fold_ln_gamma(const fvec& w, const fvec& gamma, int Co, int Cin);
 
 struct XPathPack { std::vector<half_t> g; fvec rs, cb; };
 XPathPack pack_xpath(const fvec& wn, const fvec& bn, const fvec& wi, const fvec& bi, int Cm, int Co, int Cin, int L);
diff --git a/140-extdm-distribution-extrapolation-diffusion-model-for-video-prediction_amd/csrc/runtime.cpp b/140-extdm-distribution-extrapolation-diffusion-model-for-video-prediction_amd/csrc/runtime.cpp
--- a/140-extdm-distribution-extrapolation-diffusion-model-for-video-prediction_amd/csrc/runtime.cpp
+++ b/140-extdm-distribution-extrapolation-diffusion-model-for-video-prediction_amd/csrc/runtime.cpp
@@ -634,10 +634,9 @@
       last_core = true;
       Scope sc(arena);
       const int hid = cfg.heads * cfg.dim_head;
-      View ln = alloc_cf(x.B, x.C, x.T, x.H, x.W);
-      if (!plan && bench_stage == 0) channel_ln(s, ln, x, nullptr, D(p + ".fn.norm.gamma"));
       View qkv = alloc_cf(x.B, 3 * hid, x.T, x.H, x.W);
-      if (bench_stage == 0 || bench_stage == 2) conv(qkv, ln, nullptr, P(p + ".fn.fn.attn.qkv.weight"), 1, 0, nullptr);
+      ln_conv(qkv, x, nullptr, p + ".fn.fn.attn.qkv.weight", p + ".fn.norm.gamma", nullptr, nullptr, bench_stage == 0,
+              bench_stage == 0 || bench_stage == 2);
       View o = alloc_cf(x.B, hid, x.T, x.H, x.W);
       if (!plan && (bench_stage == 0 || bench_stage == 1))
         REQUIRE(attention_core(s, qkv, o, g, cfg.heads, cfg.dim_head, bias_dense.at(p), bstride, rope_cos, rope_sin,
@@ -785,21 +784,104 @@
     return {L, ((1 << L) - 1) * tm()};
   }
 
+  const bool ln_fold = !env_flag("EXTDM_NO_LN_FOLD");
+  const bool adaptor_fold = !env_flag("EXTDM_NO_ADAPTOR_FOLD");
+  std::unordered_map<std::string, bool> fold_route;
+  template <class F>
+  bool fold_on(const std::string& key, F&& covered) {
+    auto it = fold_route.find(key);
+    if (it != fold_route.end()) return it->second;
+    return fold_route[key] = covered();
+  }
+  const PackedW& Pln(const std::string& wn, const std::string& gn) {
+    const std::string key = wn + "#ln";
+    if (!host.count(key)) {
+      const HostTensor& t = H(wn);
+      const int co = (int)t.shape[0], ci = (int)t.shape[1];
+      REQUIRE((int)H(gn).f.size() == ci && t.f.size() == (size_t)co * ci, "LayerNorm fold: 1x1 weight / gamma sizes: " + wn);
+      host[key] = HostTensor{fold_ln_gamma(t.f, H(gn).f, co, ci), {}, t.shape};
+    }
+    return P(key);
+  }
+  void ln_conv(const View& out, const View& in0, const View* in1, const std::string& wn, const std::string& gn,
+               const float* bias, const View* res, bool norm = true, bool run = true) {
+    Scope sc(arena);
+    const bool fold = ln_fold && x3_convs() && fold_on(wn + "#ln", [&] {
+      return P(wn).wx != nullptr && conv_x3_aff_covers(out, in0, in1, P(wn), 2);
+    });
+    if (!fold) {
+      View ln = alloc_cf(out.B, in0.C + (in1 ? in1->C : 0), out.T, out.H, out.W);
+      if (!plan && norm) channel_ln(s, ln, in0, in1, D(gn));
+      if (run) conv(out, ln, nullptr, P(wn), 1, 0, bias, res);
+      return;
+    }
+    const PackedW& w = Pln(wn, gn);
+    float2* st = reinterpret_cast<float2*>(arena.alloc((size_t)2 * out.B * out.T * out.HW()));
+    const size_t sbytes = conv_x3_split_bytes(out, in0, in1, w);
+    float* ws = sbytes ? arena.alloc(sbytes / sizeof(float)) : nullptr;
+    if (plan) return;
+    if (norm) channel_ln_stats(s, st, in0, in1);
+    if (!run) return;
+    ConvEpi e;
+    e.bias = bias;
+    if (res) { e.res = res->p; e.res_sb = res->sb; e.res_sc = res->sc; e.res_st = res->st; }
+    e.split_ws = ws;
+    e.split_ws_bytes = sbytes;
+    e.in_aff_mode = 2;
+    e.in_aff = st;
+    REQUIRE(conv_x3_forward(s, out, in0, in1, w, e), "LayerNorm-folded 1x1 conv: launch not covered");
+  }
+
+  int adaptor_only = 0;
+
   void adaptor(const std::string& p, const View& x) {
     Scope sc(arena);
     const int B = x.B, C = x.C, Hh = x.H, Ww = x.W, tc = tm(), tp = cfg.tp, HW = Hh * Ww;
     const AdaptorGeom ag = adaptor_geom();
     const std::string ap = p + ".adaptors";
+    const bool all = adaptor_only == 0;
     View E = alloc_tm(B, C, tc << ag.L, Hh, Ww);
     {
-      Scope s2(arena);
-      View ln = alloc_cf(B, C, tc, Hh, Ww);
       View xm = x.frames(0, tc);
-      if (!plan) channel_ln(s, ln, xm, nullptr, D(ap + ".predictor.fn.norm.gamma"));
-      conv(E.frames(0, tc), ln, nullptr, P(ap + ".predictor.fn.fn.weight"), 1, 0, D(ap + ".predictor.fn.fn.bias"),
-           &xm);
-    }
-    for (int l = 0; l < ag.L; ++l) {
+      ln_conv(E.frames(0, tc), xm, nullptr, ap + ".predictor.fn.fn.weight", ap + ".predictor.fn.norm.gamma",
+              D(ap + ".predictor.fn.fn.bias"), &xm, all, all);
+    }
+    const bool fold = adaptor_fold && x3_convs() && fold_on(p + "#extrapolators", [&] {
+      for (int l = 0; l < ag.L; ++l) {
+        const std::string wn = ap + ".extrapolators." + std::to_string(l) + ".fn.weight";
+        const int nl = tc << l;
+        if (H(wn).shape[2] != 1 || has(ap + ".extrapolators." + std::to_string(l) + ".fn.bias") || !P(wn).wx ||
+            !conv_x3_aff_covers(E.frames(nl, nl), E.frames(0, nl), nullptr, P(wn), 1))
+          return false;
+      }
+      return true;
+    });
+    if (fold) {
+      double2* carry = reinterpret_cast<double2*>(arena.alloc((size_t)4 * B * C));
+      for (int l = 0; l < ag.L; ++l) {
+        Scope s2(arena);
+        const int nl = tc << l, nc = l ? nl / 2 : nl;
+        const PackedW& w = P(ap + ".extrapolators." + std::to_string(l) + ".fn.weight");
+        float2* mr = reinterpret_cast<float2*>(arena.alloc((size_t)2 * B * C));
+        float* sd = arena.alloc((size_t)B * C);
+        const size_t sbytes = conv_x3_split_bytes(E.frames(nl, nl), E.frames(0, nl), nullptr, w);
+        float* ws = sbytes ? arena.alloc(sbytes / sizeof(float)) : nullptr;
+        if (plan) continue;
+        if (all) adaptor_stats_inc(s, E.frames(nl - nc, nc), (long)(nl - nc) * HW, carry, mr, sd);
+        if (!all && !(adaptor_only == 1 && l == ag.L - 1)) continue;
+        const View cur = E.frames(0, nl);
+        ConvEpi e;
+        e.res = cur.p; e.res_sb = cur.sb; e.res_sc = cur.sc; e.res_st = cur.st;
+        e.post_scale = sd;
+        e.post_first = 1;
+        e.split_ws = ws;
+        e.split_ws_bytes = sbytes;
+        e.in_aff_mode = 1;
+        e.in_aff = mr;
+        REQUIRE(conv_x3_forward(s, E.frames(nl, nl), cur, nullptr, w, e), "folded extrapolator conv: launch not covered");
+      }
+    }
+    for (int l = 0; l < (fold ? 0 : ag.L); ++l) {
       Scope s2(arena);
       const int nl = tc << l;
       const std::string wn = ap + ".extrapolators." + std::to_string(l) + ".fn.weight";
@@ -807,21 +889,22 @@
       float* mean = arena.alloc((size_t)B * C);
       float* sd = arena.alloc((size_t)B * C);
       View cur = E.frames(0, nl);
-      if (!plan) adaptor_stats(s, cur, mean, sd, partials);
+      const bool run = all || (adaptor_only == 1 && l == ag.L - 1);
+      if (!plan && all) adaptor_stats(s, cur, mean, sd, partials);
       if (!t3) {
         View hn = alloc_tm(B, C, nl, Hh, Ww);
-        if (!plan) adaptor_normalize(s, hn, cur, mean, sd);
-        conv(E.frames(nl, nl), hn, nullptr, P(wn), 1, 1, nullptr, &hn, ACT_NONE, sd, mean);
+        if (!plan && all) adaptor_normalize(s, hn, cur, mean, sd);
+        if (run) conv(E.frames(nl, nl), hn, nullptr, P(wn), 1, 1, nullptr, &hn, ACT_NONE, sd, mean);
       } else {
         View hp = alloc_tm(B, C, nl + 2, Hh, Ww);
         View hn = hp.frames(1, nl);
-        if (!plan) {
+        if (!plan && all) {
           zero_pad_frames(s, hp);
           adaptor_normalize(s, hn, cur, mean, sd);
         }
         View win = hp;
         win.C = 3 * C; win.T = nl;
-        conv(E.frames(nl, nl), win, nullptr, Ptime3(wn), 1, 1, nullptr, &hn, ACT_NONE, sd, mean);
+        if (run) conv(E.frames(nl, nl), win, nullptr, Ptime3(wn), 1, 1, nullptr, &hn, ACT_NONE, sd, mean);
       }
     }
     View ein = E.frames(tc, ag.F);
@@ -829,11 +912,10 @@
     View mo = alloc_tm(B, C, tp, Hh, Ww);
     View mo2 = mo;
     mo2.C = tp * C; mo2.T = 1; mo2.sc = HW; mo2.st = 0;
-    conv(mo2, ein, nullptr, P(p + ".Tmodulator.weight"), 1, 0, D(p + ".Tmodulator.bias"));
+    if (all) conv(mo2, ein, nullptr, P(p + ".Tmodulator.weight"), 1, 0, D(p + ".Tmodulator.bias"));
     View xp = x.frames(tc, tp);
-    View lnf = alloc_cf(B, 2 * C, tp, Hh, Ww);
-    if (!plan) channel_ln(s, lnf, mo, &xp, D(p + ".fuser.norm.gamma"));
-    conv(xp, lnf, nullptr, P(p + ".fuser.fn.weight"), 1, 0, D(p + ".fuser.fn.bias"), &xp);
+    ln_conv(xp, mo, &xp, p + ".fuser.fn.weight", p + ".fuser.norm.gamma", D(p + ".fuser.fn.bias"), &xp, all,
+            all || adaptor_only == 2);
   }
 
   void trajwarp_kv(const View& fea) {
@@ -2223,6 +2305,42 @@
       *flops_out = 2.0 * B * T * (double)(upl ? Li : Lo) * (upl ? Li : Lo) * (double)c_out * c_in * 16;
       return;
     }
+    if (layer == 20 || layer == 21) {
+      int lv = -1;
+      for (int i = 0; i < h->cfg.n_levels && lv < 0; ++i)
+        if (h->has("downs." + std::to_string(i) + ".4.adaptors.predictor.fn.fn.weight")) lv = i;
+      REQUIRE(lv >= 0, "bench layers 20-21: the model has no MotionAdaptor in its down path");
+      const std::string pre = "downs." + std::to_string(lv) + ".4";
+      const int C = h->cfg.dim * h->cfg.dim_mults[lv], Lq = L >> lv;
+      View x = h->alloc_cf(B, C, T, Lq, Lq);
+      fill_normal(s, x.p, 1, (int)x.numel(), 17, 0, 0, 1);
+      struct OnlyReset {
+        ExtdmHandle* h;
+        ~OnlyReset() { h->adaptor_only = 0; }
+      } only_reset{h};
+      h->adaptor(pre, x);
+      h->adaptor_only = layer == 20 ? 1 : 2;
+      note_kernel("");
+      h->adaptor(pre, x);
+      h->bench_kernel[layer] = noted_kernel();
+      hipEvent_t e0, e1;
+      HIPCHK(hipEventCreate(&e0));
+      HIPCHK(hipEventCreate(&e1));
+      HIPCHK(hipEventRecord(e0, s));
+      for (int i = 0; i < iters; ++i) h->adaptor(pre, x);
+      HIPCHK(hipEventRecord(e1, s));
+      HIPCHK(hipEventSynchronize(e1));
+      float ms = 0.f;
+      HIPCHK(hipEventElapsedTime(&ms, e0, e1));
+      (void)hipEventDestroy(e0);
+      (void)hipEventDestroy(e1);
+      *ms_out = ms / iters;
+      const AdaptorGeom ag = h->adaptor_geom();
+      const double px = (double)B * Lq * Lq;
+      *flops_out = layer == 20 ? 2.0 * px * (h->tm() << (ag.L - 1)) * (double)C * C * 9
+                               : 2.0 * px * h->cfg.tp * (double)C * 2 * C;
+      return;
+    }
     static const char* names[] = {"init_conv.weight", "downs.0.0.block2.proj.weight", "downs.1.0.block2.proj.weight",
                                   "downs.2.0.block2.proj.weight", "ups.3.0.res_conv.weight",
                                   "downs.0.0.block2.proj.weight"};
diff --git a/scripts_gpu/adaptor_fold_layers.py b/scripts_gpu/adaptor_fold_layers.py
--- /dev/null
+++ b/scripts_gpu/adaptor_fold_layers.py
@@ -0,0 +1,30 @@
+import gc
+import json
+import os
+import sys
+
+sys.path.insert(0, os.path.dirname(os.path.abspath(__file__)))
+import cfg_handle
+
+SW = ('EXTDM_NO_ADAPTOR_FOLD', 'EXTDM_NO_LN_FOLD')
+res, kern = {}, {}
+for arm in ('fold', 'separate'):
+    for k in SW:
+        os.environ.pop(k, None)
+        if arm == 'separate':
+            os.environ[k] = '1'
+    h, B, prec = cfg_handle.make('bair')
+    for k in SW:
+        os.environ.pop(k, None)
+    for rep in range(3):
+        for layer in (20, 21):
+            ms, fl = h.bench_layer(B, layer, 20)
+            kern[f'{layer}_{arm}'] = h.bench_layer_kernel(layer)
+            res.setdefault(f'{layer}_{arm}', []).append(round(ms * 1e3, 1))
+            print(f'rep {rep} layer {layer} {arm}: {ms * 1e3:.1f} us  {fl / ms / 1e9:.1f} TF/s  [{kern[f"{layer}_{arm}"]}]', flush=True)
+    del h
+    gc.collect()
+out_dir = os.environ.get('OUT', 'bench_out')
+os.makedirs(out_dir, exist_ok=True)
+print(json.dumps({'batch': B, 'us': res}))
+open(os.path.join(out_dir, 'adaptor_fold_layers.json'), 'w').write(json.dumps({'batch': B, 'us': res, 'kernel': kern}))
diff --git a/scripts_gpu/adaptor_fold_summary.py b/scripts_gpu/adaptor_fold_summary.py
--- /dev/null
+++ b/scripts_gpu/adaptor_fold_summary.py
@@ -0,0 +1,95 @@
+import csv
+import json
+import os
+import re
+import sys
+
+REPO = os.path.dirname(os.path.dirname(os.path.abspath(__file__)))
+src = sys.argv[1] if len(sys.argv) > 1 else os.path.join(REPO, os.environ.get('OUT', 'bench_out'))
+out = sys.argv[2] if len(sys.argv) > 2 else os.path.join(REPO, 'profiles', 'adaptor_fold.json')
+FORWARDS = 41.0
+PASSES = ('adaptor_stats_kernel', 'adaptor_norm_kernel', 'channel_ln4_kernel', 'channel_ln_kernel',
+          'adaptor_stats_inc_kernel', 'channel_ln_stats4_kernel', 'channel_ln_stats_kernel')
+
+
+def short(n):
+    n = n.replace('extdm::(anonymous namespace)::', '').replace('void ', '')
+    return n[:n.find('>(') + 1] if '>(' in n else n[:n.find('(')] if '(' in n else n
+
+
+def rows(path):
+    r = {}
+    for x in csv.DictReader(open(path)):
+        r[short(x['Name'])] = {'calls': int(x['Calls']), 'total_us': round(float(x['TotalDurationNs']) / 1e3, 1),
+                               'avg_us': round(float(x['AverageNs']) / 1e3, 1), 'min_us': round(float(x['MinNs']) / 1e3, 1),
+                               'max_us': round(float(x['MaxNs']) / 1e3, 1), 'stddev_us': round(float(x['StdDev']) / 1e3, 1)}
+    return r
+
+
+def last_json(path):
+    return json.loads(open(path).read().strip().splitlines()[-1])
+
+
+def workspace_gb(path):
+    m = re.search(r'"workspace_gb": ([0-9.]+)', open(path).read())
+    return float(m.group(1)) if m else None
+
+
+tr = {arm: rows(os.path.join(src, f'adaptor_fold_{arm}_kernel_stats.csv')) for arm in ('parent', 'fold')}
+res = {'command': 'scripts_gpu/adaptor_fold_ab.sh', 'per_launch': {}}
+moved = sorted(k for k in set(tr['parent']) | set(tr['fold']) if k.startswith('conv_x3_kernel<') and
+               tr['parent'].get(k, {}).get('calls', 0) != tr['fold'].get(k, {}).get('calls', 0))
+for arm in ('parent', 'fold'):
+    t = tr[arm]
+    passes = {k: t[k] for k in PASSES if k in t}
+    convs = {k: t[k] for k in moved if k in t}
+    res['per_launch'][arm] = {
+        'passes': passes, 'convs_whose_template_changed': convs,
+        'passes_ms_per_step': round(sum(v['total_us'] for v in passes.values()) / FORWARDS / 1e3, 4),
+        'convs_ms_per_step': round(sum(v['total_us'] for v in convs.values()) / FORWARDS / 1e3, 4),
+        'launches_per_step': round(sum(v['calls'] for v in list(passes.values()) + list(convs.values())) / FORWARDS, 2),
+        'all_kernels_ms_per_step': round(sum(v['total_us'] for v in t.values()) / FORWARDS / 1e3, 4)}
+p, f = res['per_launch']['parent'], res['per_launch']['fold']
+res['per_launch']['saving_ms_per_step'] = round(p['passes_ms_per_step'] + p['convs_ms_per_step'] -
+                                                f['passes_ms_per_step'] - f['convs_ms_per_step'], 4)
+lp = os.path.join(src, 'adaptor_fold_layers.json')
+if os.path.exists(lp):
+    res['bench_layers_20_21'] = json.load(open(lp))
+steps = {}
+for arm in ('parent', 'fold', 'no_adaptor', 'no_ln'):
+    vals, ws = [], None
+    for rep in range(1, 100):
+        q = os.path.join(src, f'ab_{arm}_{rep}.json')
+        if not os.path.exists(q):
+            break
+        d = last_json(q)
+        vals.append(d['ms_per_step'])
+        ws = workspace_gb(q)
+    if vals:
+        steps[arm] = {'ms_per_step': vals, 'mean': round(sum(vals) / len(vals), 4), 'spread': round(max(vals) - min(vals), 4),
+                      'workspace_gb': ws}
+
+
+def gain(a, b):
+    diff = steps[a]['mean'] - steps[b]['mean']
+    margin = 3.0 * max(steps[a]['spread'], steps[b]['spread'])
+    return {'mean_difference_ms': round(diff, 4), 'margin_ms': round(margin, 4), 'counts_as_gain': bool(diff > margin)}
+
+
+res['whole_step'] = {'command': 'bench.py --gpus 1 --steps 20 --warmup 5, arms alternating', **steps}
+if 'parent' in steps and 'fold' in steps:
+    res['whole_step']['parent_vs_fold'] = gain('parent', 'fold')
+if 'no_adaptor' in steps and 'fold' in steps:
+    res['whole_step']['adaptor_fold_alone'] = gain('no_adaptor', 'fold')
+if 'no_ln' in steps and 'fold' in steps:
+    res['whole_step']['ln_fold_alone'] = gain('no_ln', 'fold')
+res['default_generation'] = {}
+for arm in ('parent', 'fold'):
+    q = os.path.join(src, f'default_{arm}.json')
+    if os.path.exists(q):
+        d = last_json(q)
+        res['default_generation'][arm] = {'ms_per_step': d['ms_per_step'], 'value': d['value'], 'workspace_gb': workspace_gb(q)}
+json.dump(res, open(out, 'w'), indent=1)
+print(json.dumps({k: res[k] for k in ('whole_step', 'default_generation')}, indent=1))
+print({k: v for k, v in res['per_launch'].items() if k == 'saving_ms_per_step'}, p['passes_ms_per_step'], f['passes_ms_per_step'],
+      p['convs_ms_per_step'], f['convs_ms_per_step'])
```
